# SimonMacLean/NeRF-or-nothing

Hardware: AMD Instinct MI355X
Metric: train rays/sec (128 samples/ray, 8×256 MLP) at 1/2/4/8 MI355X; PSNR vs ref (higher is better)
Workload: dtype f32; 1 GPU; BASELINE configs[1]: 1024-ray global batch x 128+128 samples, 8x256 MLP fwd/bwd + Adam; global_batch=1024, rays_per_gpu=1024, micro_batch=1024, parallelism=dp1, precision=f32

## Files before the change

### include/nof.h

```cpp
#ifndef NOF_H
#define NOF_H

#include <stddef.h>
#include <stdint.h>

#ifdef __cplusplus
extern "C" {
#endif

typedef enum nof_status {
  NOF_OK = 0,
  NOF_ERR_INVALID_ARG = 1,
  NOF_ERR_HIP = 2,
  NOF_ERR_RCCL = 3,
  NOF_ERR_OOM = 4,
  NOF_ERR_UNSUPPORTED = 5
} nof_status;

#define NOF_MAX_LEVELS 4

typedef struct nof_config {
  int32_t device;
  int32_t max_rays;
  int32_t num_levels;
// ... 12 lines not shown
  int32_t precision;
  int32_t grad_buckets;
  int32_t lindisp;
  int32_t ray_shape;
  float density_bias;
  float rgb_padding;
  int32_t stop_level_grad;
  float distortion_loss_mult;
} nof_config;
size_t nof_config_size(void);

enum { NOF_RAY_CONICAL = 0, NOF_RAY_CYLINDRICAL = 1 };

enum {
  NOF_PRECISION_F32 = 0,
  NOF_PRECISION_F32_SPLIT = 1,
  NOF_PRECISION_F16X2 = 2,
  NOF_PRECISION_F32_F16SPLIT = 3,
  NOF_PRECISION_F16 = 4,
  NOF_PRECISION_F16_PRODUCTS = 5
};

void nof_config_default(nof_config* cfg);
const char* nof_last_error(void);
const char* nof_version(void);

typedef struct nof_mipnerf nof_mipnerf;
typedef struct nof_mlp nof_mlp;
typedef struct nof_adam nof_adam;
typedef struct nof_gradcalc nof_gradcalc;

typedef uint64_t (*nof_output_grad_fn)(void* user, uint64_t dev_comp_rgb, int32_t level, float loss_mult_sum,
                                       uint64_t dev_loss_mults);

nof_status nof_mipnerf_create(const nof_config* cfg, nof_mipnerf** out);
nof_status nof_mipnerf_destroy(nof_mipnerf* h);
nof_status nof_mipnerf_get_gradient(nof_mipnerf* h, int32_t n, const float* origins, const float* directions,
                                    const float* radii, const float* nears, const float* fars,
                                    const float* loss_mults, nof_output_grad_fn cb, void* cb_user,
                                    float* const** out_dev_grads);
nof_status nof_mipnerf_get_gradient_device(nof_mipnerf* h, int32_t n, const float* dev_origins,
                                           const float* dev_directions, const float* dev_radii,
                                           const float* dev_nears, const float* dev_fars,
                                           const float* dev_loss_mults, const float* dev_pixels,
                                           float loss_mult_sum, float* const** out_dev_grads);
enum { NOF_GRAD_ACCUMULATE = 1, NOF_GRAD_PUBLISH = 2 };
#define NOF_GRAD_BUCKETS 2
nof_status nof_mipnerf_get_gradient_device_ex(nof_mipnerf* h, int32_t n, const float* dev_origins,
                                              const float* dev_directions, const float* dev_radii,
                                              const float* dev_nears, const float* dev_fars,
                                              const float* dev_loss_mults, const float* dev_pixels,
                                              float loss_mult_sum, uint32_t flags, float* const** out_dev_grads);
typedef void (*nof_grad_bucket_fn)(void* user, int32_t bucket, int32_t nspans, const int64_t* span_offsets,
                                   const int64_t* span_counts);
nof_status nof_mipnerf_set_grad_buckets(nof_mipnerf* h, nof_grad_bucket_fn fn, void* user);
nof_status nof_grad_bucket_spans(int32_t bucket, const int32_t* layer_sizes, int32_t count, int64_t* offsets,
                                 int64_t* counts, int32_t* nspans);
nof_status nof_mipnerf_layer_sizes(nof_mipnerf* h, int32_t* out, int32_t cap, int32_t* count);
nof_status nof_mipnerf_mlp(nof_mipnerf* h, nof_mlp** out);
nof_status nof_mipnerf_set_rng(nof_mipnerf* h, uint64_t seed, uint32_t step, uint32_t ray_base);
nof_status nof_mipnerf_get_rng(nof_mipnerf* h, uint64_t* seed, uint32_t* step, uint32_t* ray_base);

typedef struct nof_level_view {
  int32_t n, samples;
  const float* t;
  const float* weights;
  const float* comp_rgb;
  const float* density;
  const float* rgb;
  const float* density_grad;
  const float* rgb_grad;
} nof_level_view;
nof_status nof_mipnerf_level_view(nof_mipnerf* h, int32_t level, nof_level_view* out);
nof_status nof_mipnerf_cross_view(nof_mipnerf* h, int32_t level, const float** w_grad, const float** t_grad);
nof_status nof_mipnerf_set_ray_grad(nof_mipnerf* h, int32_t enable);
nof_status nof_mipnerf_ray_grad(nof_mipnerf* h, const float** dev_o_grad, const float** dev_d_grad);
nof_status nof_mipnerf_loss(nof_mipnerf* h, float* out);
nof_status nof_mipnerf_distortion_loss(nof_mipnerf* h, float* out);
nof_status nof_mipnerf_set_interlevel_loss(nof_mipnerf* h, float mult);
nof_status nof_mipnerf_interlevel_loss(nof_mipnerf* h, float* out);
enum { NOF_CONTRACT_NONE = 0, NOF_CONTRACT_SPHERE = 1 };
nof_status nof_mipnerf_set_contraction(nof_mipnerf* h, int32_t mode);
nof_status nof_mipnerf_get_contraction(nof_mipnerf* h, int32_t* mode);
typedef struct nof_model_ext {
  uint32_t size;
  int32_t appearance_views, appearance_dim;
} nof_model_ext;
nof_status nof_mipnerf_create_ex(const nof_config* cfg, const nof_model_ext* ext, nof_mipnerf** out);
nof_status nof_mipnerf_appearance(nof_mipnerf* h, float** dev_table, float** dev_grad, int32_t* views, int32_t* dim);
nof_status nof_mipnerf_set_ray_views(nof_mipnerf* h, const int32_t* dev_view_ids);
nof_status nof_mipnerf_set_render_appearance(nof_mipnerf* h, int32_t view);
#define NOF_NUMERIC_FORWARD 1u
#define NOF_NUMERIC_DELTA 2u
nof_status nof_mipnerf_numeric_status(nof_mipnerf* h, uint32_t* flags, int32_t clear);
#define NOF_CHECK_MLP_BLOCK (1u << 0)
#define NOF_CHECK_SAMPLE_IDX (1u << 1)
#define NOF_CHECK_WGRAD_GEOM (1u << 2)
#define NOF_CHECK_GATHER (1u << 3)
#define NOF_CHECK_SELFTEST (1u << 31)
nof_status nof_device_checks(uint32_t* bits, int32_t clear);
nof_status nof_device_checks_selftest(void);

typedef struct nof_render_out {
  int32_t num_levels;
  const float* comp_rgb[NOF_MAX_LEVELS];
  const float* distance[NOF_MAX_LEVELS];
  const float* acc[NOF_MAX_LEVELS];
} nof_render_out;
nof_status nof_mipnerf_render_device(nof_mipnerf* h, int32_t n, const float* dev_origins, const float* dev_dirs,
                                     const float* dev_radii, const float* dev_nears, const float* dev_fars,
                                     int32_t randomized, int32_t white_bkgd, nof_render_out* out);

typedef struct nof_dataset nof_dataset;
typedef struct nof_batch {
  int32_t n;
  float *origins, *directions, *viewdirs;
  float *radii, *nears, *fars, *loss_mults;
  float* pixels;
  int32_t* record_index;
} nof_batch;
nof_status nof_dataset_open(const char* path, int32_t device, nof_dataset** out);
nof_status nof_dataset_open_streaming(const char* path, int32_t device, int64_t max_resident_records,
                                      nof_dataset** out);
nof_status nof_dataset_is_streaming(nof_dataset* ds, int32_t* streaming);
nof_status nof_dataset_from_host(const float* records , int64_t count, int32_t device,
                                 nof_dataset** out);
nof_status nof_dataset_count(nof_dataset* ds, int64_t* count);
nof_status nof_dataset_next(nof_dataset* ds, int32_t n, uint64_t seed, uint32_t step, uint32_t ray_base,
                            void* stream, nof_batch* out, float* loss_mult_sum);
nof_status nof_dataset_destroy(nof_dataset* ds);

nof_status nof_generate_rays(const float* host_poses, int32_t num_views, int32_t width, int32_t height, float focal,
                             float near_, float far_, int32_t ndc, const float* dev_images, float* dev_records,
                             void* stream);
nof_status nof_dataset_generate(const float* host_poses, int32_t num_views, int32_t width, int32_t height, float focal,
                                float near_, float far_, int32_t ndc, const float* dev_images, int32_t device,
                                nof_dataset** out);

nof_status nof_multiscale_layout(int32_t width, int32_t height, float focal, int32_t num_scales,
                                 int32_t disable_multiscale_loss, int32_t num_views, int32_t* w ,
                                 int32_t* h , float* focals , float* lossmults ,
                                 int64_t* firsts , int64_t* count);
nof_status nof_dataset_from_images(const float* host_poses, int32_t num_views, int32_t width, int32_t height,
                                   float focal, float near_, float far_, int32_t ndc, const float* dev_images,
                                   int32_t num_scales, int32_t disable_multiscale_loss, int32_t device,
                                   nof_dataset** out);
nof_status nof_dataset_materialize(nof_dataset* ds, float* dev_records, void* stream);
nof_status nof_recenter_poses(float* host_poses, int32_t num_views);

nof_status nof_checkpoint_save(const char* path, nof_mipnerf* h, nof_adam* adam);
nof_status nof_checkpoint_load(const char* path, nof_mipnerf* h, nof_adam* adam);

typedef struct nof_dp nof_dp;
nof_status nof_dp_unique_id(uint8_t id[128]);
nof_status nof_dp_init_rank(const uint8_t id[128], int32_t world, int32_t rank, int32_t device, nof_dp** out);
nof_status nof_dp_init_rank_timeout(const uint8_t id[128], int32_t world, int32_t rank, int32_t device,
                                    int32_t timeout_ms, nof_dp** out);
nof_status nof_dp_init_all(int32_t ndev, const int32_t* devices, nof_dp** out );
nof_status nof_dp_allreduce(nof_dp* dp, float* dev_buf, int64_t count, void* stream);
nof_status nof_dp_allreduce_grads(nof_dp* dp, nof_mipnerf* h, void* stream);
nof_status nof_dp_allreduce_grads_all(int32_t n, nof_dp* const* dps, nof_mipnerf* const* hs, void* const* streams);
nof_status nof_dp_attach(nof_dp* dp, nof_mipnerf* h, void* comm_stream);
nof_status nof_dp_wait(nof_dp* dp, int32_t timeout_ms);
nof_status nof_dp_step_end(nof_dp* dp, int32_t timeout_ms);
nof_status nof_dp_abort(nof_dp* dp);
nof_status nof_dp_destroy(nof_dp* dp);
// ... 204 lines not shown
```

### nerf-or-nothing_amd/csrc/capi.cpp

```cpp
#include <hip/hip_runtime.h>

#include <cmath>
#include <cstring>
#include <string>
#include <vector>

#include "../../include/nof.h"
#include "host/accelerated.h"
#include "host/trainer.h"
#include "host/dp.h"
#include "kernels/launch.h"

using namespace AcceleratedNeRFUtils;

struct nof_mipnerf { AcceleratedMipNeRF* impl; };
struct nof_mlp { AcceleratedMLP* impl; };
struct nof_adam { AcceleratedAdamOptimizer* impl; };
struct nof_dataset { RayDataset* impl; };
struct nof_gradcalc { AcceleratedGradientCalculator* impl; };

static thread_local std::string g_err;

template <class F>
static nof_status guard(F&& f) {
// ... 187 lines not shown
    *bits = nof::check_unit_sampling(c) | nof::check_unit_mlp_fwd16(c) | nof::check_unit_mlp_bwd16(c) |
            nof::check_unit_wgrad(c) | nof::check_unit_dataset(c) | nof::check_unit_view(c) |
            nof::check_unit_appearance(c);
#else
    (void)clear;
    throw Error(NOF_ERR_UNSUPPORTED, "device checks are compiled only into lib/libnof_check.so (make check)");
#endif
  });
}
nof_status nof_device_checks_selftest(void) {
  return guard([&] {
#ifdef NOF_DEVICE_CHECKS
    NOF_HIP(nof::launch_check_selftest(nullptr));
    NOF_HIP(hipDeviceSynchronize());
#else
    throw Error(NOF_ERR_UNSUPPORTED, "device checks are compiled only into lib/libnof_check.so (make check)");
#endif
  });
}
nof_status nof_mipnerf_set_grad_buckets(nof_mipnerf* h, nof_grad_bucket_fn fn, void* user) {
  return guard([&] {
    ARG(h);
    h->impl->mlp->set_bucket_hook(fn, user);
  });
}
static void copy_sizes(const std::vector<int>& s, int32_t* out, int32_t cap, int32_t* count) {
  if (count) *count = (int32_t)s.size();
  if (out) {
    ARG(cap >= (int32_t)s.size());
    for (size_t i = 0; i < s.size(); ++i) out[i] = s[i];
  }
}
nof_status nof_mipnerf_layer_sizes(nof_mipnerf* h, int32_t* out, int32_t cap, int32_t* count) {
  return guard([&] { ARG(h); copy_sizes(h->impl->GetLayerSizes(), out, cap, count); });
}
nof_status nof_mipnerf_mlp(nof_mipnerf* h, nof_mlp** out) {
  return guard([&] {
    ARG(h && out);
    *out = reinterpret_cast<nof_mlp*>(h->impl->mlp);
  });
}
nof_status nof_mipnerf_set_rng(nof_mipnerf* h, uint64_t seed, uint32_t step, uint32_t ray_base) {
  return guard([&] { ARG(h); h->impl->set_rng(seed, step, ray_base); });
}
nof_status nof_mipnerf_get_rng(nof_mipnerf* h, uint64_t* seed, uint32_t* step, uint32_t* ray_base) {
  return guard([&] { ARG(h && seed && step && ray_base); h->impl->get_rng(seed, step, ray_base); });
}
nof_status nof_mipnerf_level_view(nof_mipnerf* h, int32_t level, nof_level_view* out) {
  return guard([&] { ARG(h && out); *out = h->impl->level_view(level); });
}
nof_status nof_mipnerf_cross_view(nof_mipnerf* h, int32_t level, const float** w_grad, const float** t_grad) {
  return guard([&] { ARG(h && w_grad && t_grad); h->impl->cross_view(level, w_grad, t_grad); });
}
nof_status nof_mipnerf_set_ray_grad(nof_mipnerf* h, int32_t enable) {
  return guard([&] { ARG(h && (enable == 0 || enable == 1)); DEV(h); h->impl->set_ray_grad(enable != 0); });
}
nof_status nof_mipnerf_ray_grad(nof_mipnerf* h, const float** dev_o_grad, const float** dev_d_grad) {
  return guard([&] { ARG(h && dev_o_grad && dev_d_grad); h->impl->ray_grad(dev_o_grad, dev_d_grad); });
}
nof_status nof_mipnerf_loss(nof_mipnerf* h, float* out) {
  return guard([&] { ARG(h && out); DEV(h); *out = h->impl->loss(); });
}
nof_status nof_mipnerf_distortion_loss(nof_mipnerf* h, float* out) {
  return guard([&] { ARG(h && out); DEV(h); *out = h->impl->distortion_loss(); });
}
nof_status nof_mipnerf_set_interlevel_loss(nof_mipnerf* h, float mult) {
  return guard([&] {
    ARG(h);
    if (!(std::isfinite(mult) && mult >= 0.0f))
      throw Error(NOF_ERR_INVALID_ARG, "invalid argument: interlevel_loss_mult must be finite and >= 0");
    DEV(h);
    h->impl->set_interlevel_loss(mult);
  });
}
nof_status nof_mipnerf_interlevel_loss(nof_mipnerf* h, float* out) {
  return guard([&] { ARG(h && out); DEV(h); *out = h->impl->interlevel_loss(); });
}
nof_status nof_mipnerf_set_contraction(nof_mipnerf* h, int32_t mode) {
  return guard([&] {
    ARG(h && (mode == NOF_CONTRACT_NONE || mode == NOF_CONTRACT_SPHERE));
    h->impl->set_contraction(mode);
  });
}
nof_status nof_mipnerf_get_contraction(nof_mipnerf* h, int32_t* mode) {
  return guard([&] { ARG(h && mode); *mode = h->impl->contraction(); });
}
nof_status nof_mipnerf_render_device(nof_mipnerf* h, int32_t n, const float* o, const float* d, const float* radii,
                                     const float* nears, const float* fars, int32_t randomized, int32_t white_bkgd,
                                     nof_render_out* out) {
  return guard([&] {
    ARG(h && out);
    *out = nof_render_out{};
    DEV(h);
    h->impl->Render(n, o, d, radii, nears, fars, randomized, white_bkgd, out);
  });
}
nof_status nof_dataset_open(const char* path, int32_t device, nof_dataset** out) {
  return guard([&] {
    ARG(path && out);
    KEEP_DEVICE;
    auto* d = new nof_dataset{nullptr};
    try { d->impl = new RayDataset(std::string(path), device); } catch (...) { delete d; throw; }
    *out = d;
  });
}
nof_status nof_dataset_open_streaming(const char* path, int32_t device, int64_t max_resident_records,
                                      nof_dataset** out) {
  return guard([&] {
    ARG(path && out && max_resident_records >= 0);
    KEEP_DEVICE;
    auto* d = new nof_dataset{nullptr};
    try { d->impl = new RayDataset(std::string(path), device, max_resident_records); } catch (...) { delete d; throw; }
    *out = d;
  });
}
nof_status nof_dataset_is_streaming(nof_dataset* ds, int32_t* streaming) {
  return guard([&] { ARG(ds && streaming); *streaming = ds->impl->streaming() ? 1 : 0; });
}
nof_status nof_dataset_from_host(const float* records, int64_t count, int32_t device, nof_dataset** out) {
  return guard([&] {
    ARG(records && out);
    KEEP_DEVICE;
    auto* d = new nof_dataset{nullptr};
    try { d->impl = new RayDataset(records, count, device); } catch (...) { delete d; throw; }
    *out = d;
  });
}
nof_status nof_dataset_count(nof_dataset* ds, int64_t* count) {
  return guard([&] { ARG(ds && count); *count = ds->impl->count(); });
}
nof_status nof_dataset_next(nof_dataset* ds, int32_t n, uint64_t seed, uint32_t step, uint32_t ray_base, void* stream,
                            nof_batch* out, float* loss_mult_sum) {
  return guard([&] {
    ARG(ds && out);
    DEV(ds);
    ds->impl->next(n, seed, step, ray_base, (hipStream_t)stream, out, loss_mult_sum);
  });
}
nof_status nof_dataset_destroy(nof_dataset* ds) {
  return guard([&] {
    if (!ds) return;
    DEV(ds);
    delete ds->impl;
    delete ds;
  });
}
nof_status nof_generate_rays(const float* poses, int32_t V, int32_t w, int32_t h, float focal, float near_, float far_,
                             int32_t ndc, const float* dev_images, float* dev_records, void* stream) {
  return guard([&] { generate_rays(poses, V, w, h, focal, near_, far_, ndc, dev_images, dev_records, (hipStream_t)stream); });
}
nof_status nof_dataset_generate(const float* poses, int32_t V, int32_t w, int32_t h, float focal, float near_,
                                float far_, int32_t ndc, const float* dev_images, int32_t device, nof_dataset** out) {
  return guard([&] {
    ARG(poses && out);
    KEEP_DEVICE;
    auto* d = new nof_dataset{nullptr};
    try { d->impl = new RayDataset(poses, V, w, h, focal, near_, far_, ndc, dev_images, device); } catch (...) { delete d; throw; }
    *out = d;
  });
}
nof_status nof_multiscale_layout(int32_t width, int32_t height, float focal, int32_t num_scales,
                                 int32_t disable_multiscale_loss, int32_t num_views, int32_t* w, int32_t* h,
                                 float* focals, float* lossmults, int64_t* firsts, int64_t* count) {
  return guard([&] {
    ARG(w && h && focals && lossmults && firsts && count);
    const nof::MultiscaleLayout L =
// ... 602 lines not shown
```

### nerf-or-nothing_amd/csrc/host/accelerated.cpp

```cpp
#include "accelerated.h"

#include <algorithm>
#include <cmath>
#include <cstring>

#include "../kernels/common.h"
#include "../kernels/mlp_common.h"
#include "../kernels/mlp_h32.h"
#include "trace.h"

namespace AcceleratedNeRFUtils {

using nof::kBlk;

void KernelTimer::enable(uint32_t mask, hipStream_t st) {
  mask_ = mask;
  st_ = st;
  used_ = 0;
  recs_.clear();
  for (int i = 0; i < NOF_NUM_TIMERS; ++i) { tot_ms_[i] = 0.0f; tot_n_[i] = 0; }
}
void KernelTimer::fold() {
  if (!recs_.empty()) NOF_HIP(hipEventSynchronize(recs_.back().b));
  for (const Rec& r : recs_) {
// ... 119 lines not shown
}

AcceleratedMLP::AcceleratedMLP(int deg_point, int deg_view, const nof_config& cfg, int app_views, int app_dim)
    : cfg_(cfg) {
  check_model(cfg, app_views, app_dim);
  if (app_dim > 0) { gV_ = app_views; gG_ = app_dim; }
  NOF_REQUIRE(deg_point == cfg.max_deg_point - cfg.min_deg_point && deg_view == cfg.deg_view,
              "AcceleratedMLP(deg_point, deg_view) must match the config");
  NOF_HIP(hipSetDevice(cfg.device));
  st_ = (hipStream_t)cfg.stream;
  hipDeviceProp_t prop;
  NOF_HIP(hipGetDeviceProperties(&prop, cfg.device));
  num_cu_ = prop.multiProcessorCount;
  aligned_ = cfg.grad_buckets != 0;

  const int D = cfg.net_depth, W = cfg.net_width, Dc = cfg.net_depth_condition, Wc = cfg.net_width_condition;
  const int pos = 6 * (cfg.max_deg_point - cfg.min_deg_point), dir = 3 * (2 * cfg.deg_view + 1);
  const int L = D + Dc + 2;
  out_.resize(L); in_.resize(L); woff_.resize(L); boff_.resize(L);
  for (int l = 0; l < D; ++l) { out_[l] = W; in_[l] = l == 0 ? pos : (l % cfg.skip_layer == 0 ? W + pos : W); }
  out_[D] = 1; in_[D] = W;
  out_[D + 1] = Wc; in_[D + 1] = W + dir + gG_;
  for (int i = 1; i < Dc; ++i) { out_[D + 1 + i] = Wc; in_[D + 1 + i] = Wc; }
  out_[D + 1 + Dc] = 3; in_[D + 1 + Dc] = Wc;
  size_t o = 0;
  for (int l = 0; l < L; ++l) { woff_[l] = (int)o; o += (size_t)out_[l] * in_[l]; }
  for (int l = 0; l < L; ++l) { boff_[l] = (int)o; o += out_[l]; }
  NOF_REQUIRE(o < (size_t)1 << 31, "network too large");
  P_ = o;
  generic_ = any_shape(cfg);
  cross_ = cfg.stop_level_grad == 0 && cfg.num_levels > 1;

  params_.alloc(P_);
  grads_.alloc(P_);
  NOF_HIP(hipMemset(grads_.p, 0, P_ * sizeof(float)));
  std::vector<float> h(P_, 0.0f);
  glorot_host(h.data(), out_.data(), in_.data(), woff_.data(), L, cfg.seed);
  NOF_HIP(hipMemcpy(params_.p, h.data(), P_ * sizeof(float), hipMemcpyHostToDevice));
  for (int l = 0; l < L; ++l) { param_views_.push_back(params_.p + woff_[l]); grad_views_.push_back(grads_.p + woff_[l]); }
  for (int l = 0; l < L; ++l) { param_views_.push_back(params_.p + boff_[l]); grad_views_.push_back(grads_.p + boff_[l]); }

  precision_ = cfg.precision;
  numeric_.alloc(2);
  NOF_HIP(hipMemset(numeric_.p, 0, 2 * sizeof(uint32_t)));
  if (generic_) {
    gD_ = D; gW_ = W; gDc_ = Dc; gWc_ = Wc; gskip_ = cfg.skip_layer; gmin_deg_ = cfg.min_deg_point;
    gP_ = pos; gVd_ = dir;
    gen_alloc();
    return;
  }
  if (precision_ == NOF_PRECISION_F32_SPLIT) {
    wimg_f_.alloc(nof::fwd_image_split_floats<1>() + nof::kFwdTail);
    wimg_b_.alloc(nof::bwd_image_split_floats<1>() + nof::kBwdTail);
  } else if (precision_ == NOF_PRECISION_F16) {
    wimg_f_.alloc(nof::kFwdH32Floats + nof::kFwdTail);
    wimg_b_.alloc(nof::kBwdH32Floats + nof::kBwdTail);
    amax_.alloc(cfg.num_levels);
  } else if (f16_pieces()) {
    wimg_f_.alloc(nof::fwd_image_split_floats<2>() + nof::kFwdTail);
    wimg_b_.alloc(nof::bwd_image_split_floats<2>() + nof::kBwdTail);
    amax_.alloc(cfg.num_levels);
  } else {
    wimg_f_.alloc(nof::kFwdImageFloats);
    wimg_b_.alloc(nof::kBwdImageFloats);
  }

  lv_.resize(cfg.num_levels);
  for (int l = 0; l < cfg.num_levels; ++l) {
    Level& L = lv_[l];
    L.cap = cfg.max_rays * cfg.num_samples[l];
    const size_t nb = (size_t)L.cap / kBlk;
    L.act_in.alloc(nb * nof::kInF * kBlk);
    L.act_h.alloc(8 * nb * 256 * kBlk);
    L.act_h9.alloc(nb * 128 * kBlk);
    L.masks.alloc(nb * nof::kMaskSlots * 256);
    L.zhead.alloc((size_t)L.cap * 4);
    L.sigma.alloc(L.cap);
    L.rgb.alloc((size_t)L.cap * 3);
    L.delta.alloc(8 * nb * 256 * kBlk);
    L.delta9x.alloc(nb * nof::kD9F * kBlk);
    NOF_HIP(hipMemset(L.delta9x.p, 0, L.delta9x.n * sizeof(float)));
    max_M_ = std::max(max_M_, L.cap);
  }
  slab_cap_ = (size_t)(num_cu_ + 64) * 65536;
  slabs_.alloc(slab_cap_);
  bias_slabs_.alloc((size_t)(num_cu_ + 64) * 256);
}

std::vector<int> AcceleratedMLP::get_layer_sizes() const {
  const int L = num_layers();
  std::vector<int> s(2 * L);
  for (int l = 0; l < L; ++l) { s[l] = out_[l] * in_[l]; s[L + l] = out_[l]; }
  return s;
}

bool AcceleratedMLP::pack_weights(const nof::StratArgs* strat) {
  if (generic_) {
    if (f16_products()) {
      NOF_HIP(hipMemsetAsync(amax_.p, 0, lv_.size() * sizeof(uint32_t), st_));
      amax_cleared_ = (1u << lv_.size()) - 1u;
      amax_given_ = 0u;
    }
    return false;
  }
  nof::PackArgs pa;
  if (strat) pa.strat = *strat;
  for (int l = 0; l < kLayers; ++l) { pa.woff[l] = woff_[l]; pa.boff[l] = boff_[l]; }
  if (f16_pieces()) {
    pa.zero = amax_.p;
    pa.nzero = (int)lv_.size();
    amax_cleared_ = (1u << lv_.size()) - 1u;
    amax_given_ = 0u;
  }
  tb(kTPack);
  if (precision_ == NOF_PRECISION_F16)
    NOF_HIP(nof::launch_pack_weights_h32(params_.p, pa, wimg_f_.p, wimg_b_.p, st_));
  else if (precision_ != NOF_PRECISION_F32)
    NOF_HIP(nof::launch_pack_weights_x3(params_.p, pa, wimg_f_.p, wimg_b_.p, f16_pieces() ? 2 : 1, st_));
  else NOF_HIP(nof::launch_pack_weights(params_.p, pa, wimg_f_.p, wimg_b_.p, st_));
  te(kTPack);
  return strat != nullptr;
}

uint32_t* AcceleratedMLP::claim_delta_amax(int level) {
  if (!(f16_pieces() || f16_products()) || level < 0 || level >= (int)lv_.size() || !((amax_cleared_ >> level) & 1u)) return nullptr;
  amax_cleared_ &= ~(1u << level);
  amax_given_ |= 1u << level;
  return amax_.p + level;
}

void AcceleratedMLP::run_forward(int level, const nof::FwdArgs& a0) {
  Level& L = lv_[level];
  nof::FwdArgs a = a0;
  a.split = precision_;
  a.dbias = cfg_.density_bias;
  a.rgb_pad = cfg_.rgb_padding;
  a.rgb_scale = rgb_scale();
  a.wimg = wimg_f_.p;
  a.act_in = L.act_in.p;
  a.act_h = L.act_h.p;
  a.act_h9 = L.act_h9.p;
  a.masks = L.masks.p;
  a.zhead = L.zhead.p;
  a.sigma = L.sigma.p;
  a.rgb = L.rgb.p;
  tb(kTMlpFwd);
  NOF_HIP(nof::launch_mlp_fwd(a, st_));
  te(kTMlpFwd);
}

void AcceleratedMLP::forward_fused(int level, int n, int samples, const float* t, const float* origins,
                                   const float* dirs, const float* radii, bool inference) {
  NOF_REQUIRE(level >= 0 && level < (int)lv_.size(), "level out of range");
  const int M = n * samples;
  NOF_REQUIRE(n > 0 && samples % kBlk == 0 && M <= lv_[level].cap, "batch exceeds the level's capacity");
  lv_[level].M = M; lv_[level].n = n; lv_[level].S = samples;
  if (generic_) {
    NOF_REQUIRE(n <= cfg_.max_rays, "n_rays exceeds max_rays");
    GenLevel& G = gl_[level];
    tb(kTMlpFwd);
    NOF_HIP(nof::launch_cast(n, samples, t, origins, dirs, radii, G.mean.p, G.cov.p, st_, cfg_.ray_shape,
                             contraction_));
    int v;
    NOF_HIP(nof::launch_encode_g(n, samples, G.mean.p, G.cov.p, dirs, gmin_deg_, gP_, gVd_, G.enc_pos.p, G.enc_dir.p,
                                 st_, &v));
    tally(v);
    if (gG_) appearance_gather(level, n);
    te(kTMlpFwd);
    gen_forward(level, G.enc_pos.p, G.enc_dir.p);
    return;
  }
  nof::FwdArgs a{};
  a.M = M; a.S = samples; a.encoded = 0;
  a.no_store = inference ? 1 : 0;
  a.cylinder = cfg_.ray_shape == NOF_RAY_CYLINDRICAL ? 1 : 0;
  a.t = t; a.origins = origins; a.dirs = dirs; a.radii = radii;
  run_forward(level, a);
}

std::pair<float*, float*> AcceleratedMLP::get_output(const float* enc_pos, const float* enc_dir, int level,
                                                     int n_rays, int samples) {
  NOF_REQUIRE(level >= 0 && level < (int)lv_.size(), "level out of range");
  NOF_REQUIRE(enc_pos && enc_dir, "null encoded inputs");
  const int M = n_rays * samples;
  NOF_REQUIRE(n_rays > 0 && samples > 0 && samples % kBlk == 0 && M <= lv_[level].cap,
              "n_rays * samples must be a multiple of 32 within the level's capacity");
  pack_weights();
  lv_[level].M = M; lv_[level].n = n_rays; lv_[level].S = samples;
  if (generic_) {
    NOF_REQUIRE(n_rays <= cfg_.max_rays, "n_rays exceeds max_rays");
    GenLevel& G = gl_[level];
    NOF_HIP(hipMemcpyAsync(G.enc_pos.p, enc_pos, (size_t)M * gP_ * sizeof(float), hipMemcpyDeviceToDevice, st_));
    NOF_HIP(hipMemcpyAsync(G.enc_dir.p, enc_dir, (size_t)n_rays * gVd_ * sizeof(float), hipMemcpyDeviceToDevice,
                           st_));
    if (gG_) appearance_gather(level, n_rays);
    gen_forward(level, G.enc_pos.p, G.enc_dir.p);
    return {lv_[level].sigma.p, lv_[level].rgb.p};
  }
  nof::FwdArgs a{};
  a.M = M; a.S = samples; a.encoded = 1;
  a.enc_pos = enc_pos; a.enc_dir = enc_dir;
  run_forward(level, a);
  return {lv_[level].sigma.p, lv_[level].rgb.p};
}

nof_mlp_debug AcceleratedMLP::debug_view(int level) const {
  NOF_REQUIRE(level >= 0 && level < (int)lv_.size(), "level out of range");
  const Level& L = lv_[level];
  nof_mlp_debug d{};
  d.M = L.M;
  if (generic_) {
    const GenLevel& G = gl_[level];
    d.generic = 1;
    d.gen_h = G.h.p; d.gen_hc = G.hc.p; d.zhead = G.z.p;
    return d;
  }
  d.act_in = L.act_in.p; d.act_h = L.act_h.p; d.act_h9 = L.act_h9.p; d.masks = L.masks.p; d.zhead = L.zhead.p;
  d.delta = L.delta.p; d.delta9x = L.delta9x.p;
  return d;
}

int grad_bucket_spans(const int* sizes, int num_layers, int b, int64_t* off, int64_t* cnt) {
  NOF_REQUIRE(sizes && num_layers >= 1 && b >= 0 && b < AcceleratedMLP::kBuckets, "bad bucket query");
  int64_t w5 = 0, wend = 0, total = 0;
  for (int l = 0; l < num_layers; ++l) {
    if (l < 5) w5 += sizes[l];
    wend += sizes[l];
    total += sizes[l] + sizes[num_layers + l];
  }
  if (b == 0) {
    off[0] = w5; cnt[0] = wend - w5;
    return 1;
  }
  off[0] = 0; cnt[0] = w5;
  off[1] = wend; cnt[1] = total - wend;
  return 2;
}

int AcceleratedMLP::bucket_spans(int b, int64_t* off, int64_t* cnt) const {
  const std::vector<int> s = get_layer_sizes();
  return grad_bucket_spans(s.data(), num_layers(), b, off, cnt);
}

AcceleratedMLP::Schedule& AcceleratedMLP::schedule(int lv0, int lv1, int bucket) {
  NOF_REQUIRE(lv0 >= 0 && lv0 < lv1 && lv1 <= (int)lv_.size(), "bad level range");
  std::vector<int64_t> key{lv0, lv1, bucket, aligned_ ? 1 : 0};
  for (int l = lv0; l < lv1; ++l) key.push_back(lv_[l].M);
  auto it = sched_.find(key);
  if (it != sched_.end()) return it->second;
  const int nlev = lv1 - lv0;
  std::vector<nof::WgProblem> P;
  std::vector<int> pbucket;
  std::vector<int> pnblk;
  struct OutSpec { int prob, row_off, nrows, col_off, ncols; float* dst; int ld, dst_col; float* bias; };
  std::vector<OutSpec> os;
  float* G = grads_.p;
  const bool half = f16_blocks();
  auto at = [&](float* base, size_t off) -> const float* {
    return half ? reinterpret_cast<const float*>(reinterpret_cast<const uint16_t*>(base) + off) : base + off;
// ... 267 lines not shown
      const bool cleared = (amax_cleared_ >> level) & 1u;
      amax_cleared_ &= ~(1u << level);
      NOF_HIP(nof::launch_delta_amax(density_grad, color_grad, L.M, amax_.p + level, st_, numeric_.p, cleared));
    }
    b.amax = amax_.p + level;
  }
  b.dsigma = density_grad; b.drgb = color_grad; b.zhead = L.zhead.p;
  b.masks = L.masks.p;
  b.wimg_b = wimg_b_.p;
  b.delta = L.delta.p; b.delta9x = L.delta9x.p;
  return b;
}

void AcceleratedMLP::run_backward(int level, const float* color_grad, const float* density_grad) {
  const nof::BwdArgs b = bwd_args(level, color_grad, density_grad);
  tb(kTMlpBwd);
  NOF_HIP(nof::launch_mlp_bwd(b, st_));
  te(kTMlpBwd);
}

void AcceleratedMLP::run_backward2(int level, const float* const* color_grads, const float* const* density_grads) {
  nof::BwdArgs b = bwd_args(level, color_grads[0], density_grads[0]);
  const nof::BwdArgs b1 = bwd_args(level + 1, color_grads[1], density_grads[1]);
  b.M1 = b1.M; b.dsigma1 = b1.dsigma; b.drgb1 = b1.drgb; b.zhead1 = b1.zhead; b.amax1 = b1.amax;
  b.masks1 = b1.masks; b.delta1 = b1.delta; b.delta9x1 = b1.delta9x;
  tb(kTMlpBwd);
  NOF_HIP(nof::launch_mlp_bwd(b, st_));
  te(kTMlpBwd);
}

float* const* AcceleratedMLP::wgrad_levels(int lv0, int lv1, int accumulate, bool buckets) {
  if (!buckets) {
    run_wgrad(schedule(lv0, lv1), accumulate);
  } else {
    for (int bk = 0; bk < kBuckets; ++bk) {
      run_wgrad(schedule(lv0, lv1, bk), accumulate);
      int64_t off[2], cnt[2];
      const int ns = bucket_spans(bk, off, cnt);
      TraceRange hr("nof:gradient_bucket_hook");
      hook_(hook_user_, bk, ns, off, cnt);
    }
  }
  return grad_views_.data();
}

float* const* AcceleratedMLP::get_gradient(const float* color_grad, const float* density_grad, int level,
                                           uint32_t flags) {
  NOF_REQUIRE(level >= 0 && level < (int)lv_.size(), "level out of range");
  Level& L = lv_[level];
  NOF_REQUIRE(L.M > 0, "get_gradient before get_output for this level");
  NOF_REQUIRE(color_grad && density_grad, "null output gradients");
  NOF_REQUIRE((flags & ~(uint32_t)(NOF_GRAD_ACCUMULATE | NOF_GRAD_PUBLISH)) == 0, "unknown gradient flags");
  const bool buckets = (flags & NOF_GRAD_PUBLISH) && hook_;
  if (generic_) {
    gen_backward(level, color_grad, density_grad, (level > 0 || (flags & NOF_GRAD_ACCUMULATE)) ? 1 : 0);
    return gen_publish(buckets);
  }
  if (!buckets) (void)schedule(level, level + 1);
  else
    for (int b = 0; b < kBuckets; ++b) (void)schedule(level, level + 1, b);
  run_backward(level, color_grad, density_grad);
  return wgrad_levels(level, level + 1, (level > 0 || (flags & NOF_GRAD_ACCUMULATE)) ? 1 : 0, buckets);
}

float* const* AcceleratedMLP::get_gradient_levels(const float* const* color_grads, const float* const* density_grads,
                                                  uint32_t flags) {
  const int nl = (int)lv_.size();
  NOF_REQUIRE(color_grads && density_grads, "null output gradients");
  for (int l = 0; l < nl; ++l) {
    NOF_REQUIRE(lv_[l].M > 0, "get_gradient before get_output for a level");
    NOF_REQUIRE(color_grads[l] && density_grads[l], "null output gradients");
  }
  NOF_REQUIRE((flags & ~(uint32_t)(NOF_GRAD_ACCUMULATE | NOF_GRAD_PUBLISH)) == 0, "unknown gradient flags");
  const bool buckets = (flags & NOF_GRAD_PUBLISH) && hook_;
  if (generic_) {
    for (int l = 0; l < nl; ++l)
      gen_backward(l, color_grads[l], density_grads[l], (l > 0 || (flags & NOF_GRAD_ACCUMULATE)) ? 1 : 0);
    return gen_publish(buckets);
  }
  if (!buckets) (void)schedule(0, nl);
  else
    for (int b = 0; b < kBuckets; ++b) (void)schedule(0, nl, b);
  int l = 0;
  if (precision_ == NOF_PRECISION_F16)
    for (; l + 1 < nl; l += 2) run_backward2(l, color_grads + l, density_grads + l);
  for (; l < nl; ++l) run_backward(l, color_grads[l], density_grads[l]);
  return wgrad_levels(0, nl, (flags & NOF_GRAD_ACCUMULATE) ? 1 : 0, buckets);
}

static nof::GemmSrc gsrc(const float* p, int64_t si, int64_t sk, int idiv = 1) {
  nof::GemmSrc s;
  s.p = p; s.si = si; s.sk = sk; s.idiv = idiv;
  return s;
}

bool AcceleratedMLP::gen_product(nof::GemmArgs a, int ksplit, bool ws, bool f32) {
  int v;
  if (ksplit == 1) {
    a.kchunk = (a.K1 + a.K2 + 15) / 16 * 16;
    a.slab_stride = 0;
  }
  if (ws && !f16_products() && (!a.G || a.mask_in)) {
    nof::GemmArgs w = a;
    w.G = nullptr;
    if (nof::gemm_ws_fits(w)) {
      NOF_HIP(nof::launch_gemm_ws(w, st_, &v));
      tally(v);
      return true;
    }
  }
  NOF_REQUIRE(a.G || !a.mask_in, "a ReLU-bit mask needs the weight-stationary kernel");
  a.mask_in = nullptr;
  a.mask_out = nullptr;
  if (f16_products() && !f32) {
    NOF_HIP(nof::launch_gemm_h(a, ksplit, st_, &v));
    tally_h(v);
  } else {
    NOF_HIP(nof::launch_gemm(a, ksplit, st_, &v));
    tally(v);
  }
  return false;
}

void AcceleratedMLP::gen_split(int nout, int ncols, int M, int* ksplit, int* kchunk) {
  const int tiles = ((nout + 63) / 64) * ((ncols + 63) / 64);
  int ks = std::max(1, std::min((1024 + tiles - 1) / tiles, M / 64));
  const int kc = ((M + ks - 1) / ks + 15) / 16 * 16;
  *kchunk = kc;
  *ksplit = (M + kc - 1) / kc;
}

void AcceleratedMLP::gen_alloc() {
  const int NL = cfg_.num_levels;
  lv_.resize(NL);
  gl_.resize(NL);
  for (int l = 0; l < NL; ++l) {
    Level& L = lv_[l];
    GenLevel& G = gl_[l];
    L.cap = cfg_.max_rays * cfg_.num_samples[l];
    const size_t M = L.cap;
    G.mean.alloc(3 * M); G.cov.alloc(3 * M);
    G.enc_pos.alloc(M * gP_);
    G.enc_dir.alloc((size_t)cfg_.max_rays * gVd_);
    if (gG_) G.edx.alloc((size_t)cfg_.max_rays * (gVd_ + gG_));
    G.h.alloc((size_t)gD_ * M * gW_);
    G.hc.alloc((size_t)gDc_ * M * gWc_);
    G.z.alloc(4 * M);
    G.mbits.alloc((size_t)(gD_ + gDc_) * M * 4);
    G.mb_ok.assign(gD_ + gDc_, 0);
    L.sigma.alloc(M);
    L.rgb.alloc(3 * M);
    max_M_ = std::max(max_M_, L.cap);
  }
  const size_t Wm = std::max(gW_, gWc_);
  gd0_.alloc((size_t)max_M_ * Wm);
  gd1_.alloc((size_t)max_M_ * Wm);
  gdz_.alloc((size_t)max_M_ * 4);
  gray_.alloc((size_t)cfg_.max_rays * gWc_);
  if (gG_) {
    const size_t T = (size_t)gV_ * gG_;
    app_table_.alloc(T);
    app_grad_.alloc(T);
    app_step_.alloc(T);
    NOF_HIP(hipMemset(app_table_.p, 0, T * sizeof(float)));
    NOF_HIP(hipMemset(app_grad_.p, 0, T * sizeof(float)));
    gdapp_.alloc((size_t)cfg_.max_rays * gG_);
  }
// ... 376 lines not shown
  t_.resize(L); w_.resize(L); C_.resize(L); dsig_.resize(L); drgb_.resize(L); loss_rays_.resize(L);
  acc_.resize(L); dist_.resize(L);
  for (int l = 0; l < L; ++l) {
    const size_t S = cfg.num_samples[l];
    t_[l].alloc(N * (S + 1)); w_[l].alloc(N * S); C_[l].alloc(3 * N); acc_[l].alloc(N); dist_[l].alloc(N);
    dsig_[l].alloc(N * S); drgb_[l].alloc(3 * N * S); loss_rays_[l].alloc(N);
  }
  dist_rays_.alloc(N);
  cross_ = mlp->cross();
  if (cross_) {
    q_.resize(L); dtr_.resize(L); dtb_.resize(L); dt_.resize(L);
    for (int l = 0; l < L; ++l) {
      const size_t S = cfg.num_samples[l];
      if (l + 1 < L) q_[l].alloc(N * S);
      if (l >= 1) { dtr_[l].alloc(N * (S + 1)); dt_[l].alloc(N * (S + 1)); }
      if (l >= 1 && l + 1 < L) dtb_[l].alloc(N * (S + 1));
    }
  }
}

AcceleratedMipNeRF::~AcceleratedMipNeRF() {
  if (attached_dp) {
    mlp->set_bucket_hook(nullptr, nullptr);
    dp_model_destroyed(attached_dp, this);
  }
  delete mlp;
}

void AcceleratedMipNeRF::set_ray_views(const int32_t* ids) {
  NOF_REQUIRE(has_appearance(), "the model has no appearance embeddings (nof_mipnerf_create_ex)");
  mlp->set_ray_views(ids);
}

void AcceleratedMipNeRF::require_ray_views() const {
  NOF_REQUIRE(!has_appearance() || mlp->ray_views(),
              "a gradient step of an appearance model needs its ray views (nof_mipnerf_set_ray_views before every "
              "step)");
}

float* const* AcceleratedMipNeRF::GetGradient(int n, const float* origins, const float* directions,
                                              const float* radii, const float* nears, const float* fars,
                                              const float* loss_mults, nof_output_grad_fn cb, void* user) {
  NOF_REQUIRE(n > 0 && n <= cfg_.max_rays, "ray count out of range");
  NOF_REQUIRE(origins && directions && radii && nears && fars && loss_mults && cb, "null argument");
  require_ray_views();
  float msum = 0.0f;
  for (int i = 0; i < n; ++i) msum += loss_mults[i];
  NOF_HIP(hipMemcpyAsync(o_.p, origins, 3 * n * sizeof(float), hipMemcpyHostToDevice, st_));
  NOF_HIP(hipMemcpyAsync(d_.p, directions, 3 * n * sizeof(float), hipMemcpyHostToDevice, st_));
  NOF_HIP(hipMemcpyAsync(radii_.p, radii, n * sizeof(float), hipMemcpyHostToDevice, st_));
  NOF_HIP(hipMemcpyAsync(nears_.p, nears, n * sizeof(float), hipMemcpyHostToDevice, st_));
  NOF_HIP(hipMemcpyAsync(fars_.p, fars, n * sizeof(float), hipMemcpyHostToDevice, st_));
  NOF_HIP(hipMemcpyAsync(lm_.p, loss_mults, n * sizeof(float), hipMemcpyHostToDevice, st_));
  return run(n, o_.p, d_.p, radii_.p, nears_.p, fars_.p, lm_.p, nullptr, msum, cb, user, NOF_GRAD_PUBLISH);
}

float* const* AcceleratedMipNeRF::GetGradientDevice(int n, const float* o, const float* d, const float* radii,
                                                    const float* nears, const float* fars, const float* loss_mults,
                                                    const float* pixels, float msum, uint32_t flags) {
  NOF_REQUIRE(n > 0 && n <= cfg_.max_rays, "ray count out of range");
  NOF_REQUIRE(o && d && radii && nears && fars && loss_mults && pixels, "null argument");
  NOF_REQUIRE(msum > 0.0f, "loss_mult_sum must be > 0");
  NOF_REQUIRE((flags & ~(uint32_t)(NOF_GRAD_ACCUMULATE | NOF_GRAD_PUBLISH)) == 0, "unknown gradient flags");
  require_ray_views();
  return run(n, o, d, radii, nears, fars, loss_mults, pixels, msum, nullptr, nullptr, flags);
}

float* const* AcceleratedMipNeRF::run(int n, const float* o, const float* d, const float* radii, const float* nears,
                                      const float* fars, const float* lm, const float* pix, float msum,
                                      nof_output_grad_fn cb_in, void* user, uint32_t flags) {
  static const char* const kFwd[] = {"nof:level0_forward", "nof:level1_forward", "nof:level2_forward",
                                     "nof:level3_forward"};
  static const char* const kBwd[] = {"nof:backward"};
  const int L = cfg_.num_levels;
  TraceRange step_range("nof:get_gradient");
  struct ViewScope {
    AcceleratedMLP* m;
    ~ViewScope() { m->set_ray_views(nullptr); m->set_appearance_job(nullptr, 0, 0); }
  } view_scope{mlp};
  if (has_appearance()) mlp->set_appearance_job(mlp->ray_views(), (flags & NOF_GRAD_ACCUMULATE) ? 1 : 0, L);
  nof::StratArgs sa;
  sa.n = n; sa.S = cfg_.num_samples[0]; sa.nears = nears; sa.fars = fars; sa.randomized = cfg_.randomized;
  sa.lindisp = cfg_.lindisp; sa.seed = seed_; sa.step = step_; sa.ray_base = ray_base_; sa.t = t_[0].p;
  const bool sampled = mlp->pack_weights(&sa);
  for (int lv = 0; lv < L; ++lv) {
    TraceRange lr(kFwd[lv & 3]);
    const int S = cfg_.num_samples[lv];
    if (lv == 0 && !sampled) {
      timer.begin(kTSample);
      NOF_HIP(nof::launch_sample_stratified(n, S, nears, fars, cfg_.randomized, seed_, step_, 0, ray_base_,
                                            t_[0].p, st_, cfg_.lindisp));
      timer.end(kTSample);
    }
    mlp->forward_fused(lv, n, S, t_[lv].p, o, d, radii);
    const bool cb = cb_in || cross_;
    if (lv + 1 < L || cb) timer.begin(kTRenderFwd);
    if (lv + 1 < L) {
      nof::RenderPdfArgs ra{};
      ra.n = n; ra.S = S; ra.sigma = mlp->density(lv); ra.rgb = mlp->rgb(lv); ra.t = t_[lv].p; ra.d = d;
      ra.white = cfg_.white_bkgd; ra.C = C_[lv].p; ra.w = w_[lv].p; ra.nonfinite = mlp->numeric_flags();
      ra.S_out = cfg_.num_samples[lv + 1]; ra.padding = cfg_.resample_padding; ra.randomized = cfg_.randomized;
      ra.seed = seed_; ra.step = step_; ra.level = (uint32_t)(lv + 1); ra.ray_base = ray_base_; ra.t_out = t_[lv + 1].p;
      NOF_HIP(nof::launch_render_fwd_pdf(ra, st_));
    } else if (cb) {
      NOF_HIP(nof::launch_render_fwd(n, S, mlp->density(lv), mlp->rgb(lv), t_[lv].p, d, cfg_.white_bkgd, C_[lv].p,
                                     w_[lv].p, st_, nullptr, nullptr, mlp->numeric_flags()));
    }
    if (lv + 1 < L || cb) timer.end(kTRenderFwd);
  }
  struct JobScope {
    AcceleratedMLP* m;
    ~JobScope() { m->set_ray_grad_job(nullptr); }
  } job_scope{mlp};
  if (mlp->ray_grad()) {
    AcceleratedMLP::RayGradJob job;
    job.n = n; job.o = o; job.d = d; job.radius = radii;
    for (int lv = 0; lv < L; ++lv) job.t[lv] = t_[lv].p;
    mlp->set_ray_grad_job(&job);
    ray_grad_valid_ = true;
  }
  if (cross_) {
    float* const* g = run_cross(n, o, d, radii, nears, fars, lm, pix, msum, cb_in, user, flags);
    dist_valid_ = true;
    prop_valid_ = true;
    last_n_ = n;
    last_fused_ = cb_in == nullptr;
    ++step_;
    return g;
  }
  nof_output_grad_fn cb = cb_in;
  if (prop_mult_ > 0.0f && L >= 2) {
    run_interlevel(n, d, nears, fars, lm, pix, msum, cb, user);
  } else {
    nof::RenderBwdArgs ra{};
    ra.n = n; ra.d = d; ra.white = cfg_.white_bkgd; ra.pix = pix; ra.lossmult = lm; ra.msum = msum;
    ra.nonfinite = mlp->numeric_flags();
    const float dmult = cfg_.distortion_loss_mult;
    if (dmult > 0.0f) { ra.nears = nears; ra.fars = fars; ra.lindisp = cfg_.lindisp; }
    int nb = 0;
    auto flush = [&]() {
      if (!nb) return;
      timer.begin(kTRenderBwd);
      NOF_HIP(nof::launch_render_bwd(ra, nb, st_));
      timer.end(kTRenderBwd);
      nb = 0;
    };
    for (int lv = 0; lv < L; ++lv) {
      const int S = cfg_.num_samples[lv];
      const float* g = nullptr;
      if (cb) {
        g = reinterpret_cast<const float*>(cb(user, (uint64_t)(uintptr_t)C_[lv].p, lv, msum, (uint64_t)(uintptr_t)lm));
        NOF_REQUIRE(g != nullptr, "output-gradient callback returned null");
      }
      if (nb && (cb || S != ra.S || nb == nof::kRenderMaxLevels)) flush();
      ra.S = S;
      nof::RenderBwdLevel& R = ra.lv[nb++];
      R.sigma = mlp->density(lv); R.rgb = mlp->rgb(lv); R.t = t_[lv].p; R.C = C_[lv].p; R.g_ext = g;
      R.lam = lv < L - 1 ? cfg_.coarse_loss_mult : 1.0f;
      R.dsigma = dsig_[lv].p; R.drgb = drgb_[lv].p; R.loss_rays = cb ? nullptr : loss_rays_[lv].p;
      R.amax = mlp->claim_delta_amax(lv);
      R.dist_mult = lv == L - 1 ? dmult : 0.0f;
      R.dist_rays = lv == L - 1 && dmult > 0.0f ? dist_rays_.p : nullptr;
      if (lv == L - 1 && !cb) {
        ra.fwd_last = 1; ra.fwd_C = C_[lv].p; ra.fwd_w = w_[lv].p;
      }
      if (cb) flush();
    }
// ... 368 lines not shown
```

### nerf-or-nothing_amd/csrc/host/accelerated.h

```cpp
#pragma once
#include <hip/hip_runtime.h>

#include <array>
#include <map>
#include <stdexcept>
#include <string>
#include <vector>

#include "../../../include/nof.h"
#include "../kernels/launch.h"

namespace AcceleratedNeRFUtils {

struct Error : std::runtime_error {
  nof_status code;
  Error(nof_status c, const std::string& m) : std::runtime_error(m), code(c) {}
};

#define NOF_HIP(expr)                                                                                    \
  do {                                                                                                   \
    hipError_t _e = (expr);                                                                              \
    if (_e != hipSuccess)                                                                                \
      throw ::AcceleratedNeRFUtils::Error(_e == hipErrorOutOfMemory ? NOF_ERR_OOM : NOF_ERR_HIP,         \
                                          std::string(#expr) + ": " + hipGetErrorString(_e));            \
// ... 11 lines not shown
  DevBuf() = default;
  explicit DevBuf(size_t count) { alloc(count); }
  void alloc(size_t count) {
    release();
    n = count;
    if (count) NOF_HIP(hipMalloc(&p, count * sizeof(T)));
  }
  void release() {
    if (p) (void)hipFree(p);
    p = nullptr;
    n = 0;
  }
  ~DevBuf() { release(); }
  DevBuf(const DevBuf&) = delete;
  DevBuf& operator=(const DevBuf&) = delete;
  DevBuf(DevBuf&& o) noexcept : p(o.p), n(o.n) { o.p = nullptr; o.n = 0; }
  DevBuf& operator=(DevBuf&& o) noexcept {
    if (this != &o) { release(); p = o.p; n = o.n; o.p = nullptr; o.n = 0; }
    return *this;
  }
};

class KernelTimer {
 public:
  void enable(uint32_t mask, hipStream_t st);
  bool on() const { return mask_ != 0; }
  void begin(int id);
  void end(int id);
  void read(float* ms, int* launches, int cap);
  ~KernelTimer();

 private:
  hipEvent_t get();
  void fold();
  static constexpr size_t kMaxRecs = 4096;
  float tot_ms_[NOF_NUM_TIMERS] = {};
  int tot_n_[NOF_NUM_TIMERS] = {};
  uint32_t mask_ = 0;
  hipStream_t st_ = nullptr;
  std::vector<hipEvent_t> pool_;
  size_t used_ = 0;
  struct Rec { int id; hipEvent_t a, b; };
  std::vector<Rec> recs_;
  hipEvent_t open_[NOF_NUM_TIMERS] = {};
};

enum TimerId { kTPack = 0, kTSample, kTMlpFwd, kTRenderFwd, kTRenderBwd, kTMlpBwd, kTWgrad, kTWgradReduce };

class AcceleratedMLP {
 public:
  static constexpr int kLayers = 11;
  static constexpr int kTensors = 22;
  static constexpr int kMaxLayers = 16;
  int num_layers() const { return (int)out_.size(); }
  bool generic() const { return generic_; }

  AcceleratedMLP(int deg_point, int deg_view, const nof_config& cfg, int app_views = 0,
                 int app_dim = 0);
  ~AcceleratedMLP() = default;

  std::vector<int> get_layer_sizes() const;
  std::pair<float*, float*> get_output(const float* enc_pos, const float* enc_dir, int level, int n_rays,
                                       int samples);
  float* const* get_gradient(const float* color_grad, const float* density_grad, int level, uint32_t flags = 0);
  float* const* get_gradient_levels(const float* const* color_grads, const float* const* density_grads,
                                    uint32_t flags);
  static constexpr int kBuckets = 2;
  void set_bucket_hook(nof_grad_bucket_fn fn, void* user) {
    hook_ = fn;
    hook_user_ = user;
    aligned_ = fn != nullptr || cfg_.grad_buckets != 0;
  }
  bool has_bucket_hook() const { return hook_ != nullptr; }
  int bucket_spans(int b, int64_t* off, int64_t* cnt) const;

  float* const* allParams() const { return param_views_.data(); }
  float* const* allGradients() const { return grad_views_.data(); }
  float* flat_params() const { return params_.p; }
  float* flat_grads() const { return grads_.p; }
  int64_t num_params() const { return (int64_t)P_; }

  void forward_fused(int level, int n, int samples, const float* t, const float* origins, const float* dirs,
                     const float* radii, bool inference = false);
  bool pack_weights(const nof::StratArgs* strat = nullptr);
  const float* density(int level) const { return lv_[level].sigma.p; }
  const float* rgb(int level) const { return lv_[level].rgb.p; }
  KernelTimer* timer = nullptr;
  hipStream_t stream() const { return st_; }
  int device() const { return cfg_.device; }
  nof_mlp_debug debug_view(int level) const;
  const uint32_t* gen_dispatch() const { return disp_; }
  void clear_gen_dispatch() { for (uint32_t& c : disp_) c = 0; }
  const uint32_t* gen_dispatch_h() const { return disp_h_; }
  void clear_gen_dispatch_h() { for (uint32_t& c : disp_h_) c = 0; }
  uint32_t* numeric_flags() const { return numeric_.p; }
  uint32_t* claim_delta_amax(int level);
  bool cross() const { return cross_; }
  void gradient_level_cross(int level, const float* color_grad, const float* density_grad, int accumulate,
                            const float** denc);
  float* const* publish_cross(uint32_t flags) { return gen_publish((flags & NOF_GRAD_PUBLISH) && hook_); }
  const float* enc_pos(int level) const { return gl_[level].ep; }
  struct RayGradJob {
    int n = 0;
    const float *o = nullptr, *d = nullptr, *radius = nullptr;
    const float* t[NOF_MAX_LEVELS] = {};
    bool first = true;
  };
  void set_ray_grad(bool on);
  bool ray_grad() const { return ray_grad_; }
  void set_ray_grad_job(const RayGradJob* job) { rg_job_ = job ? *job : RayGradJob(); }
  const float* ray_o_grad() const { return rg_o_.p; }
  const float* ray_d_grad() const { return rg_d_.p; }
  void set_contraction(int mode);
  int contraction() const { return contraction_; }
  int appearance_views() const { return gV_; }
  int appearance_dim() const { return gG_; }
  float* appearance_table() const { return app_table_.p; }
  float* appearance_grad() const { return app_grad_.p; }
  void set_ray_views(const int32_t* ids) { app_ids_ = ids; }
  const int32_t* ray_views() const { return app_ids_; }
  void set_render_appearance(int view);
  void set_appearance_job(const int32_t* ids, int accumulate, int levels) {
    app_job_ = AppJob{ids, accumulate, levels, true};
  }

 private:
  struct AppJob {
    const int32_t* ids = nullptr;
    int accumulate = 0;
    int left = 0;
    bool first = true;
  };
  struct Schedule {
    DevBuf<nof::WgProblem> probs;
    DevBuf<nof::WgItem> items;
    DevBuf<int> item_ptr;
    DevBuf<int64_t> slab_off;
    DevBuf<nof::WgOut> outs;
    int nouts = 0, max_elems = 0, num_wg = 0;
    int lv0 = 0;
  };
  struct Level {
    int cap = 0, M = 0, n = 0, S = 0;
    DevBuf<float> act_in, act_h, act_h9, zhead, sigma, rgb;
    DevBuf<float> delta, delta9x;
    DevBuf<uint32_t> masks;
  };
  void run_forward(int level, const nof::FwdArgs& a);
  nof::BwdArgs bwd_args(int level, const float* color_grad, const float* density_grad);
  void run_backward(int level, const float* color_grad, const float* density_grad);
  void run_backward2(int level, const float* const* color_grads, const float* const* density_grads);
  Schedule& schedule(int lv0, int lv1, int bucket = -1);
  std::map<std::vector<int64_t>, Schedule> sched_;
  void run_wgrad(Schedule& sc, int accumulate);
  float* const* wgrad_levels(int lv0, int lv1, int accumulate, bool buckets);
  nof_grad_bucket_fn hook_ = nullptr;
  bool aligned_ = false;
  void* hook_user_ = nullptr;
  void tb(int id) { if (timer) timer->begin(id); }
  void te(int id) { if (timer) timer->end(id); }

  nof_config cfg_;
  hipStream_t st_;
  int num_cu_ = 256;
  int precision_ = 0;
  bool f16_pieces() const {
    return precision_ == NOF_PRECISION_F16X2 || precision_ == NOF_PRECISION_F32_F16SPLIT || precision_ == NOF_PRECISION_F16;
  }
  bool f16_products() const { return precision_ == NOF_PRECISION_F16_PRODUCTS; }
  bool f16_blocks() const { return precision_ == NOF_PRECISION_F16X2 || precision_ == NOF_PRECISION_F16; }
  float rgb_scale() const { return 1.0f + 2.0f * cfg_.rgb_padding; }
  size_t P_ = 0;
  std::vector<int> out_, in_, woff_, boff_;

  bool generic_ = false;
  int gD_ = 0, gW_ = 0, gDc_ = 0, gWc_ = 0, gskip_ = 0, gmin_deg_ = 0, gP_ = 0, gVd_ = 0;
  struct GenLevel {
    DevBuf<float> mean, cov, enc_pos, enc_dir;
    DevBuf<float> edx;
    DevBuf<float> h, hc, z;
    const float *ep = nullptr, *ed = nullptr;
    DevBuf<uint32_t> mbits;
    std::vector<char> mb_ok;
  };
  bool gen_product(nof::GemmArgs a, int ksplit = 1, bool ws = false, bool f32 = false);
  uint32_t disp_[nof::kGvCount] = {};
  uint32_t disp_h_[nof::kGhCount] = {};
  void tally(int variant, int launches = 1) { if (variant >= 0) disp_[variant] += (uint32_t)launches; }
  void tally_h(int variant) { if (variant >= 0) ++disp_h_[variant]; }
  std::vector<GenLevel> gl_;
  DevBuf<float> gd0_, gd1_, gdz_, gslab_;
  DevBuf<float> gray_;
  void gen_alloc();
  void gen_forward(int level, const float* enc_pos, const float* enc_dir);
  void gen_backward(int level, const float* color_grad, const float* density_grad, int accumulate,
                    bool want_denc = false);
  bool cross_ = false;
  DevBuf<float> gd2_, gdenc_, gdenc_part_;
  void denc_alloc(int first_level);
  bool ray_grad_ = false;
  int contraction_ = NOF_CONTRACT_NONE;
  RayGradJob rg_job_;
  DevBuf<float> gddir_, rg_o_, rg_d_;
  int gV_ = 0, gG_ = 0;
  DevBuf<float> app_table_, app_grad_;
  DevBuf<float> app_step_;
  DevBuf<float> gdapp_;
  const int32_t* app_ids_ = nullptr;
  int app_const_ = -1;
  AppJob app_job_;
  void appearance_gather(int level, int n);
  size_t* wg_need_ = nullptr;
  std::vector<nof::SlabJob> wg_jobs_;
  size_t wg_off_ = 0;
  void gen_wgrad(float* dst, int64_t ld, const float* dz, int64_t ldz, int nout, nof::GemmSrc x, int ncols, int M,
                 int accumulate, float* bias_dst = nullptr, const uint32_t* scale = nullptr);
  static void gen_split(int nout, int ncols, int M, int* ksplit, int* kchunk);
  float* const* gen_publish(bool buckets);
  DevBuf<float> params_, grads_, wimg_f_, wimg_b_;
  std::vector<float*> param_views_, grad_views_;
  std::vector<Level> lv_;
  int max_M_ = 0;
  DevBuf<float> slabs_, bias_slabs_;
  DevBuf<uint32_t> amax_;
  uint32_t amax_cleared_ = 0;
  uint32_t amax_given_ = 0;
  DevBuf<uint32_t> numeric_;
  size_t slab_cap_ = 0;
};

void dp_model_destroyed(nof_dp* dp, class AcceleratedMipNeRF* model);

int grad_bucket_spans(const int* sizes, int num_layers, int b, int64_t* off, int64_t* cnt);

void check_model(const nof_config& cfg, int app_views, int app_dim);

class AcceleratedMipNeRF {
 public:
  explicit AcceleratedMipNeRF(const nof_config& cfg, int app_views = 0, int app_dim = 0);
  ~AcceleratedMipNeRF();
  AcceleratedMLP* mlp;

  float* const* GetGradient(int n, const float* origins, const float* directions, const float* radii,
                            const float* nears, const float* fars, const float* loss_mults, nof_output_grad_fn cb,
                            void* user);
  float* const* GetGradientDevice(int n, const float* o, const float* d, const float* radii, const float* nears,
                                  const float* fars, const float* loss_mults, const float* pixels, float msum,
                                  uint32_t flags = NOF_GRAD_PUBLISH);
  std::vector<int> GetLayerSizes() const { return mlp->get_layer_sizes(); }

  void set_rng(uint64_t seed, uint32_t step, uint32_t ray_base) { seed_ = seed; step_ = step; ray_base_ = ray_base; }
  void get_rng(uint64_t* seed, uint32_t* step, uint32_t* ray_base) const { *seed = seed_; *step = step_; *ray_base = ray_base_; }
  nof_level_view level_view(int level) const;
  void cross_view(int level, const float** w_grad, const float** t_grad) const;
  void set_ray_grad(bool on);
  void ray_grad(const float** o_grad, const float** d_grad) const;
  float loss();
  float distortion_loss();
  void set_interlevel_loss(float mult);
  float interlevel_loss();
  void set_contraction(int mode) { mlp->set_contraction(mode); }
  int contraction() const { return mlp->contraction(); }
  bool has_appearance() const { return mlp->appearance_dim() > 0; }
  void set_ray_views(const int32_t* ids);
  void set_render_appearance(int view) { mlp->set_render_appearance(view); }
  void require_ray_views() const;
  uint32_t numeric_status(bool clear);
  void Render(int n, const float* o, const float* d, const float* radii, const float* nears, const float* fars,
              int randomized, int white_bkgd, nof_render_out* out);
  KernelTimer timer;
  nof_dp* attached_dp = nullptr;

 private:
  float* const* run(int n, const float* o, const float* d, const float* radii, const float* nears,
                    const float* fars, const float* lm, const float* pix, float msum, nof_output_grad_fn cb,
                    void* user, uint32_t flags);
  nof_config cfg_;
  hipStream_t st_;
  uint64_t seed_;

 public:
  const nof_config& config() const { return cfg_; }
  int device() const { return cfg_.device; }

 private:
  uint32_t step_ = 0, ray_base_ = 0;
  int last_n_ = 0;
  bool last_fused_ = false;
  bool ray_grad_valid_ = false;
  bool dist_valid_ = false;
  DevBuf<float> dist_rays_;
  float prop_mult_ = 0.0f;
  bool prop_valid_ = false;
  std::vector<DevBuf<float>> prop_rays_;
  DevBuf<float> o_, d_, radii_, nears_, fars_, lm_, pix_;
  std::vector<DevBuf<float>> t_, w_, C_, dsig_, drgb_, loss_rays_, acc_, dist_;
  void launch_interlevel_level(int n, int l, const float* lm, float msum, int accumulate);
  void run_interlevel(int n, const float* d, const float* nears, const float* fars, const float* lm, const float* pix,
                      float msum, nof_output_grad_fn cb, void* user);
  bool cross_ = false;
  std::vector<DevBuf<float>> q_, dtr_, dtb_, dt_;
  float* const* run_cross(int n, const float* o, const float* d, const float* radii, const float* nears,
// ... 51 lines not shown
```

### nerf-or-nothing_amd/csrc/kernels/adam.hip

```cpp
#include "common.h"
#include "launch.h"
#include "resample.h"
#include "mlp_common.h"
#include "mlp_h32.h"

#pragma clang fp contract(off)

namespace nof {

static int strat_blocks(const StratArgs& z) { return z.n > 0 ? (z.n * (z.S + 1) + 255) / 256 : 0; }

__global__ void k_adam(int64_t n, float* __restrict__ p, const float* __restrict__ g, float* __restrict__ m,
                       float* __restrict__ v, float lr, float inv1, float inv2) {
  const float b1 = 0.9f, b2 = 0.999f;
  for (int64_t i = (int64_t)blockIdx.x * blockDim.x + threadIdx.x; i < n; i += (int64_t)gridDim.x * blockDim.x) {
    const float gi = g[i];
    const float mi = b1 * m[i] + (1.0f - b1) * gi;
    const float vi = b2 * v[i] + (1.0f - b2) * gi * gi;
    m[i] = mi;
    v[i] = vi;
    const float mh = mi * inv1, vh = vi * inv2;
    p[i] = p[i] - lr * mh * (1.0f / sqrtf(vh + 1e-8f));
  }
}

hipError_t launch_adam(int64_t n, float* p, const float* g, float* m, float* v, float lr, float inv1, float inv2,
                       hipStream_t st) {
  if (n <= 0) return hipSuccess;
  int64_t blocks = (n + 255) / 256;
  if (blocks > 2048) blocks = 2048;
  hipLaunchKernelGGL(k_adam, dim3((unsigned)blocks), dim3(256), 0, st, n, p, g, m, v, lr, inv1, inv2);
  return hipGetLastError();
}

__device__ inline void adam_at(const AdamSegs& s, int64_t i, float*& p, const float*& g) {
  int lo = 0, hi = s.n - 1;
  while (lo < hi) {
    const int mid = (lo + hi + 1) >> 1;
    if (s.off[mid] <= i) lo = mid;
    else hi = mid - 1;
  }
  p = s.p[lo] + (i - s.off[lo]);
  g = s.g[lo] + (i - s.off[lo]);
}
__device__ inline float adam_g1(float g, float p, float wdc) { return wdc != 0.0f ? g + wdc * p : g; }
__device__ inline float adam_g2(float g1, float mv) { return mv > 0.0f ? fminf(fmaxf(g1, -mv), mv) : g1; }

template <bool MAX>
__device__ inline double adam_block_reduce(double x, double* sh) {
#pragma unroll
  for (int o = 32; o > 0; o >>= 1) {
    const double y = __shfl_xor(x, o, 64);
    x = MAX ? fmax(x, y) : x + y;
  }
  if ((threadIdx.x & 63) == 0) sh[threadIdx.x >> 6] = x;
  __syncthreads();
  return MAX ? fmax(fmax(fmax(sh[0], sh[1]), sh[2]), sh[3]) : ((sh[0] + sh[1]) + sh[2]) + sh[3];
}

__global__ __launch_bounds__(256) void k_adam_stats(int64_t n, const AdamSegs s, AdamOpts o,
                                                    double* __restrict__ part) {
  __shared__ double sh[4][4];
  double s1 = 0.0, s2 = 0.0, sp = 0.0, mx = 0.0;
  for (int64_t i = (int64_t)blockIdx.x * blockDim.x + threadIdx.x; i < n; i += (int64_t)gridDim.x * blockDim.x) {
    float* pp;
    const float* gp;
    adam_at(s, i, pp, gp);
    const float pi = *pp;
    const float g1 = adam_g1(*gp, pi, o.wdc), g2 = adam_g2(g1, o.grad_max_val);
    s1 += (double)g1 * (double)g1;
    s2 += (double)g2 * (double)g2;
    sp += (double)pi * (double)pi;
    mx = fmax(mx, (double)fabsf(g1));
  }
  s1 = adam_block_reduce<false>(s1, sh[0]);
  s2 = adam_block_reduce<false>(s2, sh[1]);
  sp = adam_block_reduce<false>(sp, sh[2]);
  mx = adam_block_reduce<true>(mx, sh[3]);
  if (threadIdx.x == 0) {
    part[0 * kAdamStatBlocks + blockIdx.x] = s1;
    part[1 * kAdamStatBlocks + blockIdx.x] = s2;
    part[2 * kAdamStatBlocks + blockIdx.x] = sp;
    part[3 * kAdamStatBlocks + blockIdx.x] = mx;
  }
}

template <bool MOD>
__global__ __launch_bounds__(256) void k_adam_opt(int64_t n, const AdamSegs s, float* __restrict__ m,
                                                  float* __restrict__ v, float lr, float inv1, float inv2, AdamOpts o,
                                                  const double* __restrict__ part, int nb, AdamStepStats* rec,
                                                  int32_t iteration) {
  __shared__ double sh[4][4];
  const float b1 = 0.9f, b2 = 0.999f;
// ... 16 lines not shown
        rec->iteration = iteration;
      }
    }
  }
  for (int64_t i = (int64_t)blockIdx.x * blockDim.x + threadIdx.x; i < n; i += (int64_t)gridDim.x * blockDim.x) {
    float* pp;
    const float* gp;
    adam_at(s, i, pp, gp);
    const float pi = *pp;
    float gi = *gp;
    if (MOD) gi = adam_g2(adam_g1(gi, pi, o.wdc), o.grad_max_val) * scale;
    const float mi = b1 * m[i] + (1.0f - b1) * gi;
    const float vi = b2 * v[i] + (1.0f - b2) * gi * gi;
    m[i] = mi;
    v[i] = vi;
    const float mh = mi * inv1, vh = vi * inv2;
    *pp = pi - lr * mh * (1.0f / sqrtf(vh + 1e-8f));
  }
}

static int adam_stat_blocks(int64_t total) {
  const int64_t b = (total + 255) / 256;
  return (int)(b < kAdamStatBlocks ? b : kAdamStatBlocks);
}
hipError_t launch_adam_stats(int64_t total, const AdamSegs& s, const AdamOpts& o, double* partials, hipStream_t st) {
  if (total <= 0) return hipSuccess;
  if (s.n < 1 || s.n > kAdamMaxSegs || s.off[0] != 0 || s.off[s.n] != total) return hipErrorInvalidValue;
  hipLaunchKernelGGL(k_adam_stats, dim3((unsigned)adam_stat_blocks(total)), dim3(256), 0, st, total, s, o, partials);
  return hipGetLastError();
}
hipError_t launch_adam_opt(int64_t total, const AdamSegs& s, float* m, float* v, float lr, float inv1, float inv2,
                           const AdamOpts& o, bool modify, const double* partials, AdamStepStats* record,
                           int32_t iteration, hipStream_t st) {
  if (total <= 0) return hipSuccess;
  if (s.n < 1 || s.n > kAdamMaxSegs || s.off[0] != 0 || s.off[s.n] != total) return hipErrorInvalidValue;
  int64_t blocks = (total + 255) / 256;
  if (blocks > 2048) blocks = 2048;
  const int nb = adam_stat_blocks(total);
  if (modify)
    hipLaunchKernelGGL(k_adam_opt<true>, dim3((unsigned)blocks), dim3(256), 0, st, total, s, m, v, lr, inv1, inv2, o,
                       partials, nb, record, iteration);
  else
    hipLaunchKernelGGL(k_adam_opt<false>, dim3((unsigned)blocks), dim3(256), 0, st, total, s, m, v, lr, inv1, inv2, o,
                       partials, nb, record, iteration);
  return hipGetLastError();
}

struct LoopPtrs { float* p[kLoopMax]; };
__global__ void k_loopback_sum(int k, LoopPtrs b, int64_t n) {
  for (int64_t i = (int64_t)blockIdx.x * blockDim.x + threadIdx.x; i < n; i += (int64_t)gridDim.x * blockDim.x) {
    float s = b.p[0][i];
    for (int j = 1; j < k; ++j) s += b.p[j][i];
    for (int j = 0; j < k; ++j) b.p[j][i] = s;
  }
}
hipError_t launch_loopback_sum(int k, float* const* bufs, int64_t n, hipStream_t st) {
  if (k < 1 || k > kLoopMax) return hipErrorInvalidValue;
  if (n <= 0) return hipSuccess;
  LoopPtrs b{};
  for (int j = 0; j < k; ++j) b.p[j] = bufs[j];
  int64_t blocks = (n + 255) / 256;
  if (blocks > 2048) blocks = 2048;
  hipLaunchKernelGGL(k_loopback_sum, dim3((unsigned)blocks), dim3(256), 0, st, k, b, n);
  return hipGetLastError();
}

__device__ inline int layer_out(int l) { return l < 8 ? 256 : (l == 8 ? 1 : (l == 9 ? 128 : 3)); }
__device__ inline int layer_in(int l) {
  return l == 0 ? 96 : (l == 4 ? 352 : (l < 8 ? 256 : (l == 8 ? 256 : (l == 9 ? 283 : 128))));
}

__device__ inline void fwd_slice(int s, int& l, int& col) {
  if (s < 3) { l = 0; col = 32 * s; }
  else if (s < 27) { l = 1 + (s - 3) / 8; col = 32 * ((s - 3) % 8); }
  else if (s < 38) { l = 4; col = 32 * (s - 27); }
  else if (s < 62) { l = 5 + (s - 38) / 8; col = 32 * ((s - 38) % 8); }
  else { l = 9; col = 32 * (s - 62); }
}
__device__ inline void bwd_slice(int s, int& l, int& o) {
  if (s < 4) { l = 9; o = 32 * s; }
  else { l = 7 - (s - 4) / 8; o = 32 * ((s - 4) % 8); }
}

__global__ void k_pack_weights(const float* __restrict__ P, PackArgs pa, float* __restrict__ wf,
                               float* __restrict__ wb) {
  if ((int)blockIdx.x >= pa.pack_blocks) {
    const StratArgs& z = pa.strat;
    stratified_t(((int)blockIdx.x - pa.pack_blocks) * (int)blockDim.x + (int)threadIdx.x, z.n, z.S, z.nears, z.fars,
                 z.randomized, z.lindisp, z.seed, z.step, 0, z.ray_base, z.t);
    return;
  }
  const int64_t gid = (int64_t)blockIdx.x * blockDim.x + threadIdx.x;
  const int64_t nf = (int64_t)kFwdImageFloats, nb = (int64_t)kBwdImageFloats;
  if (gid < nf) {
    const int64_t slices = (int64_t)kFwdSlices * kSliceFloats;
    float v = 0.0f;
    if (gid < slices) {
      const int s = (int)(gid / kSliceFloats);
      const int e = (int)(gid - (int64_t)s * kSliceFloats);
      const int r = e >> 5, pc = e & 31;
      const int c = ((((pc >> 2) ^ ((r >> 1) & 7)) << 2) | (pc & 3));
      int l, col;
      fwd_slice(s, l, col);
      const int in = layer_in(l);
      if (r < layer_out(l) && col + c < in) v = P[pa.woff[l] + (int64_t)r * in + col + c];
    } else {
      const int t = (int)(gid - slices);
      if (t < kFwdTailW8) {
        const int l = t / 256, x = t % 256;
        v = x < layer_out(l) ? P[pa.boff[l] + x] : 0.0f;
      } else if (t < kFwdTailW10) {
        v = P[pa.woff[8] + (t - kFwdTailW8)];
      } else if (t < kFwdTailW9d) {
        v = P[pa.woff[10] + (t - kFwdTailW10)];
      } else {
        const int o = (t - kFwdTailW9d) / 32, k = (t - kFwdTailW9d) % 32;
        v = k < kDirIn ? P[pa.woff[9] + (int64_t)o * 283 + 256 + k] : 0.0f;
      }
    }
    wf[gid] = v;
  } else if (gid < nf + nb) {
    const int64_t b = gid - nf;
    const int64_t slices = (int64_t)kBwdSlices * kSliceFloats;
    float v = 0.0f;
    if (b < slices) {
      const int s = (int)(b / kSliceFloats);
      const int e = (int)(b - (int64_t)s * kSliceFloats);
      const int i = e >> 5, pc = e & 31;
      const int c = ((((pc >> 2) ^ ((i >> 1) & 7)) << 2) | (pc & 3));
      int l, o;
      bwd_slice(s, l, o);
      v = P[pa.woff[l] + (int64_t)(o + c) * layer_in(l) + i];
    } else {
      const int t = (int)(b - slices);
      v = t < kBwdTailW10 ? P[pa.woff[8] + t] : P[pa.woff[10] + (t - kBwdTailW10)];
    }
    wb[b] = v;
  }
}

__device__ inline float fwd_tail_value(const float* __restrict__ P, const PackArgs& pa, int t) {
  if (t < kFwdTailW8) {
    const int l = t / 256, x = t % 256;
    return x < layer_out(l) ? P[pa.boff[l] + x] : 0.0f;
  }
  if (t < kFwdTailW10) return P[pa.woff[8] + (t - kFwdTailW8)];
  if (t < kFwdTailW9d) return P[pa.woff[10] + (t - kFwdTailW10)];
  const int o = (t - kFwdTailW9d) / 32, k = (t - kFwdTailW9d) % 32;
  return k < kDirIn ? P[pa.woff[9] + (int64_t)o * 283 + 256 + k] : 0.0f;
}
__device__ inline float bwd_tail_value(const float* __restrict__ P, const PackArgs& pa, int t) {
  return t < kBwdTailW10 ? P[pa.woff[8] + t] : P[pa.woff[10] + (t - kBwdTailW10)];
}
template <int P>
__device__ inline typename SplitMode<P>::V2 split_piece2(float w, int piece) {
  typename SplitMode<P>::V2 o[SplitMode<P>::NP];
  split2<P>(w, w, o);
  typename SplitMode<P>::V2 r = o[0];
#pragma unroll
  for (int p = 1; p < SplitMode<P>::NP; ++p) r = piece == p ? o[p] : r;
  return r;
}

template <int P>
__global__ void k_pack_weights_x3(const float* __restrict__ P_, PackArgs pa, float* __restrict__ wf,
                                  float* __restrict__ wb) {
  if ((int)blockIdx.x >= pa.pack_blocks) {
    const StratArgs& z = pa.strat;
    stratified_t(((int)blockIdx.x - pa.pack_blocks) * (int)blockDim.x + (int)threadIdx.x, z.n, z.S, z.nears, z.fars,
                 z.randomized, z.lindisp, z.seed, z.step, 0, z.ray_base, z.t);
    return;
  }
  constexpr int NP = SplitMode<P>::NP;
  constexpr int kChunks = split_slice_floats<P>() / 4;
  const float* __restrict__ Pp = P_;
  const int64_t gid = (int64_t)blockIdx.x * blockDim.x + threadIdx.x;
  if (gid < pa.nzero) pa.zero[gid] = 0u;
  const int64_t nfc = (int64_t)kFwdSlices * kChunks, nbc = (int64_t)kBwdSlices * kChunks;
  if (gid < nfc + nbc) {
    const bool fwd = gid < nfc;
    const int64_t c = fwd ? gid : gid - nfc;
    const int slice = (int)(c / kChunks), q = (int)(c % kChunks);
    const int lane = q & 63, rest = q >> 6;
    const int piece = P == 2 ? rest / 16 : rest % NP, so = P == 2 ? rest % 16 : rest / NP;
    const int row = P == 2 ? 16 * so + (lane & 15) : (so & 7) * 32 + (lane & 31);
    int l, base;
    if (fwd) fwd_slice(slice, l, base);
    else bwd_slice(slice, l, base);
    const int in = layer_in(l);
    typename SplitMode<P>::V8 out;
#pragma unroll
    for (int j = 0; j < 8; ++j) {
      const int kf = P == 2 ? 16 * (j >> 2) + 4 * (lane >> 4) + (j & 3)
                            : 16 * (so >> 3) + 8 * (j >> 2) + 4 * (lane >> 5) + (j & 3);
      float w;
      if (fwd) w = (row < layer_out(l) && base + kf < in) ? Pp[pa.woff[l] + (int64_t)row * in + base + kf] : 0.0f;
      else w = Pp[pa.woff[l] + (int64_t)(base + kf) * in + row];
      out[j] = split_piece2<P>(w, piece)[0];
    }
    float* dst = (fwd ? wf : wb) + (size_t)slice * split_slice_floats<P>() + (size_t)q * 4;
    *reinterpret_cast<typename SplitMode<P>::V8*>(dst) = out;
  } else {
    const int t = (int)(gid - nfc - nbc);
    if (t < kFwdTail) wf[fwd_image_split_floats<P>() + t] = fwd_tail_value(Pp, pa, t);
    else if (t < kFwdTail + kBwdTail)
      wb[bwd_image_split_floats<P>() + (t - kFwdTail)] = bwd_tail_value(Pp, pa, t - kFwdTail);
  }
}
hipError_t launch_pack_weights_x3(const float* params, const PackArgs& pa, float* wimg_f, float* wimg_b,
                                  int precision, hipStream_t st) {
  const int chunks = precision == 2 ? split_slice_floats<2>() / 4 : split_slice_floats<1>() / 4;
  const int64_t total = (int64_t)(kFwdSlices + kBwdSlices) * chunks + kFwdTail + kBwdTail;
  PackArgs a = pa;
  a.pack_blocks = (int)((total + 255) / 256);
  const dim3 grid((unsigned)(a.pack_blocks + strat_blocks(pa.strat)));
  if (precision == 2) hipLaunchKernelGGL(k_pack_weights_x3<2>, grid, dim3(256), 0, st, params, a, wimg_f, wimg_b);
  else hipLaunchKernelGGL(k_pack_weights_x3<1>, grid, dim3(256), 0, st, params, a, wimg_f, wimg_b);
  return hipGetLastError();
}

__global__ void k_pack_weights_h32(const float* __restrict__ P, PackArgs pa, float* __restrict__ wf,
                                   float* __restrict__ wb) {
  if ((int)blockIdx.x >= pa.pack_blocks) {
    const StratArgs& z = pa.strat;
    stratified_t(((int)blockIdx.x - pa.pack_blocks) * (int)blockDim.x + (int)threadIdx.x, z.n, z.S, z.nears, z.fars,
                 z.randomized, z.lindisp, z.seed, z.step, 0, z.ray_base, z.t);
    return;
  }
  const int64_t gid = (int64_t)blockIdx.x * blockDim.x + threadIdx.x;
  if (gid < pa.nzero) pa.zero[gid] = 0u;
  const int64_t nfc = (int64_t)(kFwdFrags + kStreamPad) * 64, nbc = (int64_t)(kBwdFrags + kStreamPad) * 64;
  if (gid < nfc + nbc) {
    const bool fwd = gid < nfc;
    const int64_t q = fwd ? gid : gid - nfc;
    const int g = (int)(q >> 6), lane = (int)(q & 63), x = lane & 31, h = lane >> 5;
    f16x8 out;
#pragma unroll
    for (int j = 0; j < 8; ++j) out[j] = (_Float16)0.0f;
    if (g < (fwd ? kFwdFrags : kBwdFrags)) {
      int start = 0, si = 0;
      H32Seg sg = fwd ? fwd_seg(0) : bwd_seg(0);
      while (g >= start + sg.nk * sg.nc) {
        start += sg.nk * sg.nc;
        ++si;
        sg = fwd ? fwd_seg(si) : bwd_seg(si);
      }
      const int c = (g - start) / sg.nk, kk = (g - start) % sg.nk, l = sg.layer, in = layer_in(l);
#pragma unroll
      for (int j = 0; j < 8; ++j) {
        float w;
        if (fwd) {
          const int col = kk < 16 ? kfeat(kk, h, j) : 256 + kfeat(kk - 16, h, j);
          const bool dens = l == 9 && c == 4;
          const int ll = dens ? 8 : l, row = dens ? x : 32 * c + x;
          w = row < layer_out(ll) ? P[pa.woff[ll] + (int64_t)row * layer_in(ll) + col] : 0.0f;
        } else if (kk < 16 && (l != 9 || kk < 8)) {
          w = P[pa.woff[l] + (int64_t)kfeat(kk, h, j) * in + 32 * c + x];
        } else {
          w = (kk == 8 && kfeat(0, h, j) == 0) ? P[pa.woff[8] + 32 * c + x] : 0.0f;
        }
        out[j] = (_Float16)w;
      }
    }
    *reinterpret_cast<f16x8*>((fwd ? wf : wb) + (size_t)q * 4) = out;
  } else {
    const int t = (int)(gid - nfc - nbc);
    if (t < kFwdTail) wf[kFwdH32Floats + t] = fwd_tail_value(P, pa, t);
    else if (t < kFwdTail + kBwdTail) wb[kBwdH32Floats + (t - kFwdTail)] = bwd_tail_value(P, pa, t - kFwdTail);
  }
}
hipError_t launch_pack_weights_h32(const float* params, const PackArgs& pa, float* wimg_f, float* wimg_b,
                                   hipStream_t st) {
  const int64_t total = (int64_t)(kFwdFrags + kBwdFrags + 2 * kStreamPad) * 64 + kFwdTail + kBwdTail;
  PackArgs a = pa;
  a.pack_blocks = (int)((total + 255) / 256);
  hipLaunchKernelGGL(k_pack_weights_h32, dim3((unsigned)(a.pack_blocks + strat_blocks(pa.strat))), dim3(256), 0, st,
                     params, a, wimg_f, wimg_b);
  return hipGetLastError();
}

hipError_t launch_pack_weights(const float* params, const PackArgs& pa, float* wimg_f, float* wimg_b, hipStream_t st) {
  const int64_t total = (int64_t)kFwdImageFloats + (int64_t)kBwdImageFloats;
  PackArgs a = pa;
  a.pack_blocks = (int)((total + 255) / 256);
  hipLaunchKernelGGL(k_pack_weights, dim3((unsigned)(a.pack_blocks + strat_blocks(pa.strat))), dim3(256), 0, st,
                     params, a, wimg_f, wimg_b);
  return hipGetLastError();
}

}
```

### nerf-or-nothing_amd/csrc/kernels/launch.h

```cpp
#pragma once
#include <hip/hip_runtime.h>
#include <stdint.h>

namespace nof {

uint32_t check_unit_sampling(bool clear);
uint32_t check_unit_mlp_fwd16(bool clear);
uint32_t check_unit_mlp_bwd16(bool clear);
uint32_t check_unit_wgrad(bool clear);
uint32_t check_unit_dataset(bool clear);
uint32_t check_unit_view(bool clear);
uint32_t check_unit_appearance(bool clear);
hipError_t launch_check_selftest(hipStream_t st);

hipError_t launch_sample_stratified(int n, int S, const float* nears, const float* fars, int randomized,
                                    uint64_t seed, uint32_t step, uint32_t level, uint32_t ray_base, float* t,
                                    hipStream_t st, int lindisp = 0);
hipError_t launch_sample_pdf(int n, int S_in, const float* t_in, const float* w, int S_out, float padding,
                             int randomized, uint64_t seed, uint32_t step, uint32_t level, uint32_t ray_base,
                             float* t_out, int32_t* idx_out, hipStream_t st);
hipError_t launch_cast(int n, int S, const float* t, const float* o, const float* d, const float* radius,
                       float* mean, float* cov, hipStream_t st, int ray_shape = 0, int contraction = 0);
hipError_t launch_encode(int n, int S, const float* mean, const float* cov, const float* d, float* enc_pos,
                         float* enc_dir, hipStream_t st);
// ... 27 lines not shown
  uint32_t* amax;
  float dist_mult = 0.0f;
  float* dist_rays = nullptr;
};
struct RenderBwdArgs {
  int n, S, white;
  const float *d, *pix, *lossmult;
  float msum;
  uint32_t* nonfinite;
  RenderBwdLevel lv[kRenderMaxLevels];
  int fwd_last = 0;
  float *fwd_C = nullptr, *fwd_w = nullptr;
  const float *nears = nullptr, *fars = nullptr;
  int lindisp = 0;
};
hipError_t launch_render_bwd(const RenderBwdArgs& a, int nlev, hipStream_t st);
hipError_t launch_output_gradient(int n, const float* C, const float* pix, const float* lossmult,
                                  float loss_mult_sum, float lam, float* g, hipStream_t st);

struct RenderBwdXArgs {
  int n, S, white;
  const float *d, *pix, *lossmult;
  float msum;
  uint32_t* nonfinite;
  const float *sigma, *rgb, *t, *C, *g_ext;
  float lam;
  float *dsigma, *drgb, *loss_rays;
  const float* q;
  float* t_grad;
  int fwd;
  float *fwd_C, *fwd_w;
  float dist_mult;
  float* dist_rays;
  const float *nears, *fars;
  int lindisp;
};
hipError_t launch_render_bwd_x(const RenderBwdXArgs& a, hipStream_t st);

struct EncodeGradArgs {
  int n, S, P, min_deg, cylinder;
  const float *t, *o, *d, *radius, *enc, *denc;
  const float *add0, *add1;
  float* t_grad;
  int contract;
};
hipError_t launch_encode_grad(const EncodeGradArgs& a, hipStream_t st);
struct SamplePdfGradArgs {
  int n, S_in, S_out;
  const float *t_in, *w;
  float padding;
  int randomized;
  uint64_t seed;
  uint32_t step, level, ray_base;
  const float* t_out_grad;
  float *w_grad, *t_in_grad;
};
hipError_t launch_sample_pdf_grad(const SamplePdfGradArgs& a, hipStream_t st);

struct InterlevelArgs {
  int n, S_prop, S_tgt, accumulate;
  const float *t_prop, *w_prop, *t_tgt, *w_tgt, *lossmult;
  float msum, mult;
  float *w_grad, *rays;
};
hipError_t launch_interlevel(const InterlevelArgs& a, hipStream_t st);

struct RayGradArgs {
  int n, S, P, min_deg, cylinder, Vd, accumulate;
  const float *t, *o, *d, *radius, *enc, *denc, *sigma, *dsigma;
  const float *enc_dir, *ddir;
  float *o_grad, *d_grad;
  int contract;
};
hipError_t launch_ray_grad(const RayGradArgs& a, hipStream_t st);

struct FwdArgs {
  int M, S, encoded;
  int no_store;
  int split;
  int cylinder;
  float dbias = -1.0f, rgb_scale = 1.002f, rgb_pad = 0.001f;
  const float *t, *origins, *dirs, *radii;
  const float *enc_pos, *enc_dir;
  const float* wimg;
  float* act_in;
  float* act_h;
  float* act_h9;
  uint32_t* masks;
  float* zhead;
  float* sigma;
  float* rgb;
};
hipError_t launch_mlp_fwd(const FwdArgs& a, hipStream_t st);

struct BwdArgs {
  int M;
  int split;
  const float *dsigma, *drgb, *zhead;
  const uint32_t* amax;
  float dbias = -1.0f, rgb_scale = 1.002f;
  const uint32_t* masks;
  const float* wimg_b;
  float* delta;
  float* delta9x;
  int M1;
  const float *dsigma1, *drgb1, *zhead1;
  const uint32_t *amax1, *masks1;
  float *delta1, *delta9x1;
};
hipError_t launch_mlp_bwd(const BwdArgs& a, hipStream_t st);
hipError_t launch_delta_amax(const float* dsigma, const float* drgb, int M, uint32_t* amax, hipStream_t st,
                             uint32_t* nonfinite = nullptr, bool cleared = false);
hipError_t launch_mlp_fwd16(const FwdArgs& a, hipStream_t st);
hipError_t launch_mlp_bwd16(const BwdArgs& a, hipStream_t st);
hipError_t launch_mlp_fwd_h32(const FwdArgs& a, hipStream_t st);
int device_cus();
hipError_t launch_mlp_bwd_h32(const BwdArgs& a, hipStream_t st);

struct WgProblem {
  const float* A; const float* B;
  int FA, a_row0, ntr;
  int FB, b_col0, ntc;
  int shape;
  int ntc1;
  const float* B2; int FB2, b2_col0, ntc2;
  const float* B3; int FB3, b3_col0, ntc3;
  int level;
};
struct WgItem { int prob, kb0, kb1; int slab; };
int wgrad_reduce_threads(int nrows, int ncols, int col_off);
constexpr int kWgMaxLevels = 4;
struct WgOut {
  int item0, nitems;
  int lev_items[kWgMaxLevels];
  int nlev;
  int row_off, nrows, col_off, ncols;
  float* dst; int ld, dst_col;
  float* bias_dst;
  int prob;
};
hipError_t launch_wgrad(const WgProblem* probs, const WgItem* items, const int* item_ptr, int num_wg,
                        const int64_t* slab_off, float* slabs, float* bias_slabs, hipStream_t st);
int wgrad_shape(int ntr, int ntc, int* cost2);
int wgrad_block_cost(int ntr, int ntc, int* shape);
int wgrad_x3_grid_cols();
hipError_t launch_wgrad_x3(const WgProblem* probs, const WgItem* items, const int* item_ptr, int num_wg,
                           const int64_t* slab_off, float* slabs, float* bias_slabs, int precision, hipStream_t st);
hipError_t launch_wgrad_reduce(const WgOut* outs, int nouts, int max_elems, const WgItem* items,
                               const WgProblem* probs, const int64_t* slab_off, const float* slabs,
                               const float* bias_slabs, int accumulate, const uint32_t* amax, hipStream_t st);

struct GemmSrc {
  const float* p = nullptr;
  int64_t si = 0, sk = 0;
  int idiv = 1;
};
struct GemmArgs {
  int M = 0, N = 0, K1 = 0, K2 = 0;
  GemmSrc A1, A2, B1, B2;
  const float* bias = nullptr;
  int relu = 0;
  const float* G = nullptr; int64_t gi = 0, gj = 0;
  float* C = nullptr; int64_t ci = 0, cj = 0;
  int kchunk = 0; int64_t slab_stride = 0;
  float* rowsum = nullptr;
  const uint32_t* mask_in = nullptr;
// ... 71 lines not shown
  int64_t first[kMaxScales];
  int64_t count;
};
hipError_t launch_pyramid_level(float* pyr, const MultiscaleLayout& L, int s, hipStream_t st);
hipError_t launch_materialize(const float* poses, const float* pyr, const MultiscaleLayout& L, float near, float far,
                              int ndc, float* records, hipStream_t st);
hipError_t launch_gather_rays(const float* poses, const float* pyr, const MultiscaleLayout& L, float near, float far,
                              int ndc, int n, uint64_t seed, uint32_t step, uint32_t ray_base, float* o, float* d,
                              float* vd, float* radius, float* nears, float* fars, float* lm, float* pix, int* idx_out,
                              float* lm_sum, hipStream_t st);
hipError_t launch_pose_grad(const MultiscaleLayout& L, int n, const int* idx, const float* o_grad, const float* d_grad,
                            float* pose_grad, int accumulate, hipStream_t st);
hipError_t launch_batch_views(const MultiscaleLayout& L, int n, const int* idx, int* views, hipStream_t st);

hipError_t launch_appearance_gather(int n, int vd, int dim, int views, const float* enc_dir, const float* table,
                                    const int* ids, int const_view, float* out, hipStream_t st);
hipError_t launch_appearance_grad(int n, int dim, int views, const int* ids, const float* d_app, const float* partial,
                                  float* d_table, int accumulate, hipStream_t st);

struct ViewRayArgs {
  const float* poses;
  float pose[12];
  int use_pose, view, num_views;
  int w, h;
  float focal, near, far;
  int ndc, p0, n;
  float *o, *d, *radius, *nears, *fars;
};
hipError_t launch_view_rays(const ViewRayArgs& a, hipStream_t st);
constexpr int kViewMaxLevels = 4;
constexpr int kViewStoreBlock = 256;
inline int view_store_blocks(int n) { return (n + kViewStoreBlock - 1) / kViewStoreBlock; }
struct ViewStoreArgs {
  int num_levels;
  const float* comp_rgb[kViewMaxLevels];
  const float *dist_in, *acc_in;
  float* rgb[kViewMaxLevels];
  float *distance, *acc;
  const float* gt;
  double* partials;
  int block0, blocks;
  int p0, n, npix;
  int view, num_views;
};
hipError_t launch_view_store(const ViewStoreArgs& a, hipStream_t st);
hipError_t launch_view_final(const double* partials, int blocks, int num_levels, double* sums, hipStream_t st);

hipError_t image_metrics(const float* a, const float* b, int W, int H, float max_val, float* psnr, float* ssim,
                         hipStream_t st);

constexpr int kLoopMax = 8;
hipError_t launch_loopback_sum(int k, float* const* bufs, int64_t n, hipStream_t st);
hipError_t launch_adam(int64_t n, float* p, const float* g, float* m, float* v, float lr, float inv1, float inv2,
                       hipStream_t st);
constexpr int kAdamStatBlocks = 256;
constexpr int kAdamMaxSegs = 64;
struct AdamSegs {
  int n = 0;
  int64_t off[kAdamMaxSegs + 1] = {};
  float* p[kAdamMaxSegs] = {};
  const float* g[kAdamMaxSegs] = {};
};
struct AdamOpts {
  float grad_max_norm = 0.0f, grad_max_val = 0.0f;
  float wdc = 0.0f;
};
struct AdamStepStats {
  float weight_l2, grad_norm, grad_abs_max, grad_norm_clipped, clip_scale;
  int32_t iteration;
};
hipError_t launch_adam_stats(int64_t total, const AdamSegs& s, const AdamOpts& o, double* partials, hipStream_t st);
hipError_t launch_adam_opt(int64_t total, const AdamSegs& s, float* m, float* v, float lr, float inv1, float inv2,
                           const AdamOpts& o, bool modify, const double* partials, AdamStepStats* record,
                           int32_t iteration, hipStream_t st);
struct StratArgs {
  int n = 0, S = 0;
  const float* nears = nullptr;
  const float* fars = nullptr;
  int randomized = 0, lindisp = 0;
  uint64_t seed = 0;
  uint32_t step = 0, ray_base = 0;
  float* t = nullptr;
};
struct PackArgs {
  int woff[11]; int boff[11];
  uint32_t* zero = nullptr; int nzero = 0;
  StratArgs strat;
  int pack_blocks = 0;
};
hipError_t launch_pack_weights(const float* params, const PackArgs& pa, float* wimg_f, float* wimg_b, hipStream_t st);
hipError_t launch_pack_weights_h32(const float* params, const PackArgs& pa, float* wimg_f, float* wimg_b,
                                   hipStream_t st);
hipError_t launch_pack_weights_x3(const float* params, const PackArgs& pa, float* wimg_f, float* wimg_b,
                                  int precision, hipStream_t st);

}
```

### nerf-or-nothing_amd/csrc/kernels/mlp_bwd16.hip

```cpp
#include "common.h"
#include "launch.h"
#include "mlp16.h"

namespace nof {


template <bool kDensity, class ST, bool kSplit = false>
struct BwdEpi16 {
  static constexpr int kVmPerPart = 4;
  const f32x4 (&acc)[16];
  float (&bin)[16][4];
  const ST& bst;
  const int g;
  const float* w8;
  float dzs;
  __amdgpu_buffer_rsrc_t dst_blk;
  uint2 mk;
  f32x4 wnext;

  __device__ __forceinline__ BwdEpi16(const f32x4 (&acc_)[16], float (&bin_)[16][4], const ST& bst_, int lane)
      : acc(acc_), bin(bin_), bst(bst_), g(lane >> 4) {}
  template <class E>
  __device__ __forceinline__ void begin(const uint2* mask, E* dst_blk_, const float* w8_ = nullptr, float dzs_ = 0.0f) {
    mk = *mask;
    dst_blk = blk_rsrc_t(dst_blk_);
    if constexpr (kDensity) {
      w8 = w8_ + 4 * g;
      dzs = dzs_;
      wnext = *reinterpret_cast<const f32x4*>(w8);
    }
  }
  __device__ __forceinline__ void operator()(int t) {
    f32x4 w4;
    if constexpr (kDensity) {
      w4 = wnext;
      if (t + 1 < 16) wnext = *reinterpret_cast<const f32x4*>(w8 + 16 * (t + 1));
    }
    float v[4];
#pragma unroll
    for (int r = 0; r < 4; ++r) {
      v[r] = acc[t][r];
      if constexpr (kDensity) v[r] = __builtin_fmaf(w4[r], dzs, v[r]);
      v[r] = mask16_apply(mk, t, r, v[r]);
    }
    put_tile<kSplit, true>(bin, t, v, bst, dst_blk);
  }
  __device__ __forceinline__ void tile01() {
    (*this)(0);
    (*this)(1);
  }
};

template <int P>
__global__ __launch_bounds__(kMlp16Threads, 1) void k_mlp_bwd16(BwdArgs a) {
  typedef typename Store16<P, true>::T ST;
  typedef typename Store16<P, true>::E AE;
  __shared__ __attribute__((aligned(16))) float lds[ring16_floats<P>() + 256];
  float* w8_lds = lds + ring16_floats<P>();
  const int tid = threadIdx.x, lane = tid & 63, g = lane >> 4, j = lane & 15;
  const int wave = __builtin_amdgcn_readfirstlane(tid >> 6);
  const int half = wave & 1;
  const ST bst(lane, half);
  const int nblk = a.M / kBlk;
  const int blk_raw = blockIdx.x * 4 + (wave >> 1);
  const int blk = blk_raw < nblk ? blk_raw : nblk - 1;
  const int m = blk * kBlk + 16 * half + j;
  NOF_DCHECK(a.M % kBlk == 0 && blk >= 0 && blk < nblk, kChkMlpBlock);
  const float* tail = a.wimg_b + (size_t)kBwdSlices * kSliceFloats;
  const size_t layer_stride = (size_t)nblk * kWidth * kBlk;
  uint32_t* masks = const_cast<uint32_t*>(a.masks);

  ring16_prologue(a.wimg_b, lds, tid);

  const f32x4 zh = reinterpret_cast<const f32x4*>(a.zhead)[m];
  float dzs = a.dsigma[m] * sigmoid_f(zh[0] + a.dbias);
  float dzc[3];
#pragma unroll
  for (int c = 0; c < 3; ++c) {
    const float s = sigmoid_f(zh[1 + c]);
    dzc[c] = a.drgb[(size_t)m * 3 + c] * (s * (1.0f - s)) * a.rgb_scale;
  }
  if constexpr (P >= 2) {
    const float sc = delta_scale(a.amax, false);
    dzs *= sc;
#pragma unroll
    for (int c = 0; c < 3; ++c) dzc[c] *= sc;
  }
  const __amdgpu_buffer_rsrc_t d9 = blk_rsrc_t(reinterpret_cast<AE*>(a.delta9x) + (size_t)blk * kD9F * kBlk);
#pragma unroll
  for (int r = 0; r < 4; ++r) bst.store(d9, 8, r, g == 0 ? (r == 0 ? dzs : dzc[r - 1]) : 0.0f);
  float bin[16][4];
  {
    const uint2 mk = *mask16_ptr(masks, blk, 8, half, lane);
    const float* w10 = tail + kBwdTailW10;
#pragma unroll
    for (int t = 0; t < 8; ++t) {
      const int fb = 16 * t + 4 * g;
      const f32x4 wa = *reinterpret_cast<const f32x4*>(w10 + fb);
      const f32x4 wb = *reinterpret_cast<const f32x4*>(w10 + 128 + fb);
      const f32x4 wc = *reinterpret_cast<const f32x4*>(w10 + 256 + fb);
      float v[4];
#pragma unroll
      for (int r = 0; r < 4; ++r)
        v[r] = mask16_apply(mk, t, r, __builtin_fmaf(wc[r], dzc[2], __builtin_fmaf(wb[r], dzc[1], wa[r] * dzc[0])));
      put_tile<P >= 2, true>(bin, t, v, bst, d9);
    }
  }
  if (tid < 64) reinterpret_cast<f32x4*>(w8_lds)[tid] = reinterpret_cast<const f32x4*>(tail + kBwdTailW8)[tid];
  __syncthreads();

  int cur = 0;
  const float* wsrc = a.wimg_b;
  f32x4 accA[16], accB[16];
  AE* delta_blk = reinterpret_cast<AE*>(a.delta) + (size_t)blk * kWidth * kBlk;
  BwdEpi16<true, ST, P >= 2> e7(accA, bin, bst, lane);
  e7.begin(mask16_ptr(masks, blk, 7, half, lane), delta_blk + 7 * layer_stride, w8_lds, dzs);
  layer16<P, 4, 0, 16>(bin, nullptr, accA, lds, cur, wsrc, false, tid, lane);
  e7.tile01();
  BwdEpi16<false, ST, P >= 2> ea(accA, bin, bst, lane), eb(accB, bin, bst, lane);
  eb.begin(mask16_ptr(masks, blk, 6, half, lane), delta_blk + 6 * layer_stride);
  layer16<P, 8, 0, 16>(bin, nullptr, accB, lds, cur, wsrc, false, tid, lane, e7);
  eb.tile01();
  static_assert(kDepth == 8, "bwd pairing assumes 8 trunk layers");
  for (int l = kDepth - 2; l >= 2; l -= 2) {
    ea.begin(mask16_ptr(masks, blk, l - 1, half, lane), delta_blk + (l - 1) * layer_stride);
    layer16<P, 8, 0, 16>(bin, nullptr, accA, lds, cur, wsrc, false, tid, lane, eb);
    ea.tile01();
    eb.begin(mask16_ptr(masks, blk, l - 2, half, lane), delta_blk + (l - 2) * layer_stride);
    layer16<P, 8, 0, 16>(bin, nullptr, accB, lds, cur, wsrc, l == 2, tid, lane, ea);
    eb.tile01();
  }
#pragma unroll
  for (int t = 2; t < 16; ++t) eb(t);
}

hipError_t launch_mlp_bwd16(const BwdArgs& a, hipStream_t st) {
  const int nblk = a.M / kBlk;
  if (a.split == 2) hipLaunchKernelGGL(k_mlp_bwd16<2>, dim3((nblk + 3) / 4), dim3(kMlp16Threads), 0, st, a);
  else if (a.split == 3) hipLaunchKernelGGL(k_mlp_bwd16<3>, dim3((nblk + 3) / 4), dim3(kMlp16Threads), 0, st, a);
  else hipLaunchKernelGGL(k_mlp_bwd16<0>, dim3((nblk + 3) / 4), dim3(kMlp16Threads), 0, st, a);
  return hipGetLastError();
}

NOF_CHECK_UNIT(check_unit_mlp_bwd16)

}
```

### nerf-or-nothing_amd/csrc/kernels/mlp_fwd16.hip

```cpp
#include "common.h"
#include "geometry.h"
#include "launch.h"
#include "mlp16.h"

namespace nof {


template <bool store, bool kDensity, int NT, class ST, bool kSplit = false>
struct FwdEpi16 {
  static constexpr int kVmPerPart = store ? 4 : 0;
  const f32x4 (&acc)[16];
  float (&bin)[16][4];
  const ST& bst;
  const int g;
  const float* w8;
  __amdgpu_buffer_rsrc_t act_blk;
  uint2* mask_dst;
  uint32_t mw[2];
  f32x4 wnext;
  float zs;

  __device__ __forceinline__ FwdEpi16(const f32x4 (&acc_)[16], float (&bin_)[16][4], const ST& bst_, int lane)
      : acc(acc_), bin(bin_), bst(bst_), g(lane >> 4) {}
  template <class E>
  __device__ __forceinline__ void begin(E* act_blk_, uint2* mask_dst_, const float* w8_ = nullptr) {
    act_blk = blk_rsrc_t(act_blk_);
    mask_dst = mask_dst_;
    mw[0] = mw[1] = 0u;
    if constexpr (kDensity) {
      w8 = w8_ + 4 * g;
      wnext = *reinterpret_cast<const f32x4*>(w8);
      zs = 0.0f;
    }
  }
  __device__ __forceinline__ void operator()(int t) {
    const bool more = t + 1 < NT;
    f32x4 w4;
    if constexpr (kDensity) {
      w4 = wnext;
      if (more) wnext = *reinterpret_cast<const f32x4*>(w8 + 16 * (t + 1));
    }
    float hv[4];
#pragma unroll
    for (int r = 0; r < 4; ++r) {
      hv[r] = relu_bit(acc[t][r], mw[t >> 3]);
      if constexpr (kDensity) zs = __builtin_fmaf(w4[r], hv[r], zs);
    }
    put_tile<kSplit, store>(bin, t, hv, bst, act_blk);
    if constexpr (store && kVmPerPart > 0)
      if (!more) *mask_dst = make_uint2(mw[0], mw[1]);
  }
  __device__ __forceinline__ void tile01() {
    (*this)(0);
    (*this)(1);
  }
};

template <int P, bool store>
__global__ __launch_bounds__(kMlp16Threads, 1) void k_mlp_fwd16(FwdArgs a) {
  typedef typename Store16<P, false>::T ST;
  typedef typename Store16<P, false>::E AE;
  constexpr int kRing = ring16_slots<P>() * kSliceFloats;
  constexpr bool kIpeReg = ring16_slots<P>() == 4;
  constexpr int kIpeLds = kIpeReg ? 0 : 8 * kIpe16Floats;
  constexpr int kBiasLds = 8 * 256 + 256;
  __shared__ __attribute__((aligned(16))) float lds[kRing + kIpeLds + 8 * 128 + kBiasLds];
  const int tid = threadIdx.x, lane = tid & 63, g = lane >> 4, j = lane & 15;
  const int wave = __builtin_amdgcn_readfirstlane(tid >> 6);
  const int half = wave & 1;
  const int nblk = a.M / kBlk;
  const int blk_raw = blockIdx.x * 4 + (wave >> 1);
  const int blk = blk_raw < nblk ? blk_raw : nblk - 1;
  const int m0 = blk * kBlk;
  const int ray = m0 / a.S;
  const int s0 = m0 - ray * a.S + 16 * half;
  const int m = m0 + 16 * half + j;
  const float* tail = a.wimg + (size_t)kFwdSlices * kSliceFloats;
  NOF_DCHECK(a.M % kBlk == 0 && a.S % kBlk == 0 && blk >= 0 && blk < nblk, kChkMlpBlock);

  ring16_prologue(a.wimg, lds, tid);

  float ipe[6][4];
  float d3[3];
  if (!a.encoded) {
    d3[0] = a.dirs[3 * ray]; d3[1] = a.dirs[3 * ray + 1]; d3[2] = a.dirs[3 * ray + 2];
    const float o3[3] = {a.origins[3 * ray], a.origins[3 * ray + 1], a.origins[3 * ray + 2]};
    const float* tr = a.t + (size_t)ray * (a.S + 1) + s0 + j;
    float mean[3], cov[3];
    frustum_gaussian(tr[0], tr[1], o3, d3, a.radii[ray], mean, cov, a.cylinder != 0);
#pragma unroll
    for (int t = 0; t < 6; ++t)
#pragma unroll
      for (int r = 0; r < 4; ++r)
        ipe[t][r] = ipe_feature(feat16(t, g, r), mean, cov);
  } else {
#pragma unroll
    for (int t = 0; t < 6; ++t)
#pragma unroll
      for (int r = 0; r < 4; ++r) ipe[t][r] = a.enc_pos[(size_t)m * kPosIn + feat16(t, g, r)];
  }
  const int kl = lane < kDirIn ? lane : 0;
  const float pe_l = a.encoded ? a.enc_dir[(size_t)ray * kDirIn + kl] : dir_feature(kl, d3);
  float pe[kDirIn];
#pragma unroll
  for (int k = 0; k < kDirIn; ++k) pe[k] = __int_as_float(__builtin_amdgcn_readlane(__float_as_int(pe_l), k));

  const ST bst(lane, half);
  if constexpr (store) {
    const __amdgpu_buffer_rsrc_t act_in_rs = blk_rsrc_t(reinterpret_cast<AE*>(a.act_in) + (size_t)blk * kInF * kBlk);
#pragma unroll
    for (int t = 0; t < 6; ++t)
#pragma unroll
      for (int r = 0; r < 4; ++r) bst.store(act_in_rs, t, r, ipe[t][r]);
#pragma unroll
    for (int t = 6; t < 8; ++t)
#pragma unroll
      for (int r = 0; r < 4; ++r) {
        const int k = feat16(t, g, r) - kPosIn;
        float v = 0.0f;
#pragma unroll
        for (int kk = 0; kk < kDirIn; ++kk) v = (kk == k) ? pe[kk] : v;
        bst.store(act_in_rs, t, r, v);
      }
  }
  const float* ipe_b = &ipe[0][0];
  if constexpr (!kIpeReg) {
    float* ipe_lds = lds + kRing + wave * kIpe16Floats;
#pragma unroll
    for (int t = 0; t < 6; ++t) {
      f32x4 v;
      v[0] = ipe[t][0]; v[1] = ipe[t][1]; v[2] = ipe[t][2]; v[3] = ipe[t][3];
      *reinterpret_cast<f32x4*>(ipe_lds + (t * 64 + lane) * 4) = v;
    }
    ipe_b = ipe_lds;
  }
  float* dirb = lds + kRing + kIpeLds + wave * 128;
  float* bias_lds = lds + kRing + kIpeLds + 8 * 128;
  for (int i = tid; i < kBiasLds / 4; i += kMlp16Threads) {
    const float* src = i < 512 ? tail + kFwdTailBias + 4 * i : tail + kFwdTailW8 + 4 * (i - 512);
    *reinterpret_cast<f32x4*>(bias_lds + 4 * i) = *reinterpret_cast<const f32x4*>(src);
  }
#pragma unroll
  for (int rep = 0; rep < 2; ++rep) {
    const int o = lane + 64 * rep;
    float s = tail[kFwdTailBias + 9 * 256 + o];
    const float* w9 = tail + kFwdTailW9d + o * 32;
#pragma unroll
    for (int k = 0; k < kDirIn; ++k) s = __builtin_fmaf(w9[k], pe[k], s);
    dirb[o] = s;
  }
  __syncthreads();

  int cur = 0;
  const float* wsrc = a.wimg;
  f32x4 accA[16], accB[16];
  float bin[16][4];
  const size_t layer_stride = (size_t)nblk * kWidth * kBlk;
  const float* biases = bias_lds;
  AE* act_h_blk = reinterpret_cast<AE*>(a.act_h) + (size_t)blk * kWidth * kBlk;

  constexpr bool kPre = P >= 2;
  FwdEpi16<store, false, 16, ST, kPre> ea(accA, bin, bst, lane), eb(accB, bin, bst, lane);
  const float* bias_g = biases + 4 * g;
  ea.begin(act_h_blk, mask16_ptr(a.masks, blk, 0, half, lane));
  layer16<P, 0, 3, 16>(bin, ipe_b, accA, lds, cur, wsrc, false, tid, lane, bias_g);
  ea.tile01();
  for (int l = 1; l < kDepth - 1; l += 2) {
    eb.begin(act_h_blk + l * layer_stride, mask16_ptr(a.masks, blk, l, half, lane));
    layer16<P, 8, 0, 16>(bin, ipe_b, accB, lds, cur, wsrc, false, tid, lane, ea, bias_g + l * 256);
    eb.tile01();
    ea.begin(act_h_blk + (l + 1) * layer_stride, mask16_ptr(a.masks, blk, l + 1, half, lane));
    if (l + 1 == kSkip)
      layer16<P, 8, 3, 16>(bin, ipe_b, accA, lds, cur, wsrc, false, tid, lane, eb, bias_g + (l + 1) * 256);
    else layer16<P, 8, 0, 16>(bin, ipe_b, accA, lds, cur, wsrc, false, tid, lane, eb, bias_g + (l + 1) * 256);
    ea.tile01();
  }
  static_assert(kDepth == 8 && kSkip % 2 == 0, "trunk pairing assumes 8 layers and an even skip layer");
  FwdEpi16<store, true, 16, ST, kPre> e7(accB, bin, bst, lane);
  e7.begin(act_h_blk + 7 * layer_stride, mask16_ptr(a.masks, blk, 7, half, lane), bias_lds + 8 * 256);
  layer16<P, 8, 0, 16>(bin, ipe_b, accB, lds, cur, wsrc, false, tid, lane, ea, bias_g + 7 * 256);
  e7.tile01();

  layer16<P, 8, 0, 8>(bin, ipe_b, accA, lds, cur, wsrc, true, tid, lane, e7, dirb + 4 * g);
  float zs = e7.zs;
  zs += __shfl_xor(zs, 16, 64);
  zs += __shfl_xor(zs, 32, 64);
  zs += tail[kFwdTailBias + 8 * 256];
  FwdEpi16<store, false, 8, ST> e9(accA, bin, bst, lane);
  e9.begin(reinterpret_cast<AE*>(a.act_h9) + (size_t)blk * kWidthCond * kBlk, mask16_ptr(a.masks, blk, 8, half, lane));
#pragma unroll
  for (int t = 0; t < 8; ++t) e9(t);

  float zc[3] = {0.0f, 0.0f, 0.0f};
#pragma unroll
  for (int c = 0; c < 3; ++c) {
#pragma unroll
    for (int t = 0; t < 8; ++t) {
      const f32x4 w4 = *reinterpret_cast<const f32x4*>(tail + kFwdTailW10 + c * 128 + 16 * t + 4 * g);
#pragma unroll
      for (int r = 0; r < 4; ++r) zc[c] = __builtin_fmaf(w4[r], bin[t][r], zc[c]);
    }
    zc[c] += __shfl_xor(zc[c], 16, 64);
    zc[c] += __shfl_xor(zc[c], 32, 64);
    zc[c] += tail[kFwdTailBias + 10 * 256 + c];
  }

  if (g == 0) {
    a.sigma[m] = softplus_f(zs + a.dbias);
#pragma unroll
    for (int c = 0; c < 3; ++c) a.rgb[(size_t)m * 3 + c] = sigmoid_f(zc[c]) * a.rgb_scale - a.rgb_pad;
    f32x4 zh;
    zh[0] = zs; zh[1] = zc[0]; zh[2] = zc[1]; zh[3] = zc[2];
    if constexpr (store) reinterpret_cast<f32x4*>(a.zhead)[m] = zh;
  }
}

hipError_t launch_mlp_fwd16(const FwdArgs& a, hipStream_t st) {
  const int nblk = a.M / kBlk;
  const dim3 grid((nblk + 3) / 4), block(kMlp16Threads);
  if (a.split == 2) {
    if (a.no_store) hipLaunchKernelGGL((k_mlp_fwd16<2, false>), grid, block, 0, st, a);
    else hipLaunchKernelGGL((k_mlp_fwd16<2, true>), grid, block, 0, st, a);
  } else if (a.split == 3) {
    if (a.no_store) hipLaunchKernelGGL((k_mlp_fwd16<2, false>), grid, block, 0, st, a);
    else hipLaunchKernelGGL((k_mlp_fwd16<3, true>), grid, block, 0, st, a);
  } else {
    if (a.no_store) hipLaunchKernelGGL((k_mlp_fwd16<0, false>), grid, block, 0, st, a);
    else hipLaunchKernelGGL((k_mlp_fwd16<0, true>), grid, block, 0, st, a);
  }
  return hipGetLastError();
}

NOF_CHECK_UNIT(check_unit_mlp_fwd16)

// ... 2 lines not shown
```

### nerf-or-nothing_amd/nof/__init__.py

```python
from ._lib import NofError, default_config, lib
from .api import (
    AcceleratedAdamOptimizer,
    AcceleratedGradientCalculator,
    AcceleratedMipNeRF,
    AcceleratedMLP,
    OutputRetriever,
    RayDataset,
    load_checkpoint,
    recenter_poses,
    save_checkpoint,
    device_checks,
    device_checks_selftest,
    device_count,
    device_tensor,
    gen_dispatch_h_names,
    gen_dispatch_names,
    generate_rays,
    grad_bucket_spans,
    image_metrics,
    kernel_gemm_h,
    kernel_interlevel,
    learning_rate_decay,
    multiscale_layout,
    to_numpy,
)
```

### nerf-or-nothing_amd/nof/_lib.py

```python
from __future__ import annotations

import ctypes as C
import os

_PKG = os.path.dirname(os.path.dirname(os.path.abspath(__file__)))
LIB_PATH = os.environ.get("NOF_LIB") or os.path.join(_PKG, "lib", "libnof.so")

NOF_MAX_LEVELS = 4
NOF_NUM_TIMERS = 8
TIMER_NAMES = ("pack", "sample", "mlp_fwd", "render_fwd", "render_bwd", "mlp_bwd", "wgrad", "wgrad_reduce")
STATUS = {0: "NOF_OK", 1: "NOF_ERR_INVALID_ARG", 2: "NOF_ERR_HIP", 3: "NOF_ERR_RCCL", 4: "NOF_ERR_OOM",
          5: "NOF_ERR_UNSUPPORTED"}


class NofError(RuntimeError):
    def __init__(self, status: int, where: str, msg: str):
        super().__init__(f"{where}: {STATUS.get(status, status)}: {msg}")
        self.status = status


NOF_PRECISION_F32, NOF_PRECISION_F32_SPLIT, NOF_PRECISION_F16X2, NOF_PRECISION_F32_F16SPLIT, NOF_PRECISION_F16 = 0, 1, 2, 3, 4
NOF_PRECISION_F16_PRODUCTS = 5
PRECISION_NAMES = {"f32": NOF_PRECISION_F32, "split": NOF_PRECISION_F32_SPLIT, "f16x2": NOF_PRECISION_F16X2,
                   "f16split": NOF_PRECISION_F32_F16SPLIT, "f16": NOF_PRECISION_F16,
# ... 44 lines not shown


class nof_gemm_src(C.Structure):
    _fields_ = [("p", C.c_void_p), ("si", C.c_int64), ("sk", C.c_int64), ("idiv", C.c_int32)]


class nof_gemm_args(C.Structure):
    _fields_ = [("M", C.c_int32), ("N", C.c_int32), ("K1", C.c_int32), ("K2", C.c_int32),
                ("A1", nof_gemm_src), ("A2", nof_gemm_src), ("B1", nof_gemm_src), ("B2", nof_gemm_src),
                ("bias", C.c_void_p), ("relu", C.c_int32), ("G", C.c_void_p), ("gi", C.c_int64), ("gj", C.c_int64),
                ("C", C.c_void_p), ("ci", C.c_int64), ("cj", C.c_int64), ("kchunk", C.c_int32),
                ("slab_stride", C.c_int64), ("rowsum", C.c_void_p), ("scale_amax", C.c_void_p),
                ("scale_src", C.c_int32), ("ksplit", C.c_int32)]


class nof_render_out(C.Structure):
    _fields_ = [("num_levels", C.c_int32), ("comp_rgb", C.c_void_p * NOF_MAX_LEVELS),
                ("distance", C.c_void_p * NOF_MAX_LEVELS), ("acc", C.c_void_p * NOF_MAX_LEVELS)]


class nof_batch(C.Structure):
    _fields_ = [("n", C.c_int32)] + [(k, C.c_void_p) for k in (
        "origins", "directions", "viewdirs", "radii", "nears", "fars", "loss_mults", "pixels", "record_index")]


class nof_step_stats(C.Structure):
    _fields_ = [(k, C.c_float) for k in ("weight_l2", "grad_norm", "grad_abs_max", "grad_norm_clipped",
                                         "clip_scale")] + [("iteration", C.c_int32)]


class nof_view_out(C.Structure):
    _fields_ = [("rgb", C.c_void_p * NOF_MAX_LEVELS), ("distance", C.c_void_p), ("acc", C.c_void_p)]


class nof_view_metrics(C.Structure):
    _fields_ = [("width", C.c_int32), ("height", C.c_int32), ("num_levels", C.c_int32),
                ("mse", C.c_double * NOF_MAX_LEVELS), ("psnr", C.c_float * NOF_MAX_LEVELS), ("ssim", C.c_float)]


NOF_VIEW_SSIM = 1

OUTPUT_GRAD_FN = C.CFUNCTYPE(C.c_uint64, C.c_void_p, C.c_uint64, C.c_int32, C.c_float, C.c_uint64)
GRAD_BUCKET_FN = C.CFUNCTYPE(None, C.c_void_p, C.c_int32, C.c_int32, C.POINTER(C.c_int64), C.POINTER(C.c_int64))
NOF_GRAD_ACCUMULATE, NOF_GRAD_PUBLISH, NOF_GRAD_BUCKETS = 1, 2, 2
NOF_NUMERIC_FORWARD, NOF_NUMERIC_DELTA = 1, 2

P = C.c_void_p
F = C.c_float
I32 = C.c_int32
U32 = C.c_uint32
U64 = C.c_uint64
PP = C.POINTER(C.POINTER(C.c_float))

SIGNATURES = {
    "nof_config_default": [C.POINTER(nof_config)],
    "nof_last_error": [],
    "nof_version": [],
    "nof_config_size": [],
    "nof_mipnerf_create": [C.POINTER(nof_config), C.POINTER(P)],
    "nof_mipnerf_create_ex": [C.POINTER(nof_config), C.POINTER(nof_model_ext), C.POINTER(P)],
    "nof_mipnerf_appearance": [P, C.POINTER(P), C.POINTER(P), C.POINTER(I32), C.POINTER(I32)],
    "nof_mipnerf_set_ray_views": [P, P],
    "nof_mipnerf_set_render_appearance": [P, I32],
    "nof_mipnerf_destroy": [P],
    "nof_mipnerf_get_gradient": [P, I32, P, P, P, P, P, P, OUTPUT_GRAD_FN, P, C.POINTER(PP)],
    "nof_mipnerf_get_gradient_device": [P, I32, P, P, P, P, P, P, P, F, C.POINTER(PP)],
    "nof_mipnerf_get_gradient_device_ex": [P, I32, P, P, P, P, P, P, P, F, U32, C.POINTER(PP)],
    "nof_mipnerf_set_grad_buckets": [P, GRAD_BUCKET_FN, P],
    "nof_grad_bucket_spans": [I32, C.POINTER(I32), I32, C.POINTER(C.c_int64), C.POINTER(C.c_int64),
                              C.POINTER(I32)],
    "nof_mipnerf_layer_sizes": [P, C.POINTER(I32), I32, C.POINTER(I32)],
    "nof_mipnerf_mlp": [P, C.POINTER(P)],
    "nof_mipnerf_set_rng": [P, U64, U32, U32],
    "nof_mipnerf_get_rng": [P, C.POINTER(U64), C.POINTER(U32), C.POINTER(U32)],
    "nof_mipnerf_level_view": [P, I32, C.POINTER(nof_level_view)],
    "nof_mipnerf_cross_view": [P, I32, C.POINTER(P), C.POINTER(P)],
    "nof_mipnerf_set_ray_grad": [P, I32],
    "nof_mipnerf_ray_grad": [P, C.POINTER(P), C.POINTER(P)],
    "nof_mipnerf_loss": [P, C.POINTER(F)],
    "nof_mipnerf_distortion_loss": [P, C.POINTER(F)],
    "nof_mipnerf_set_interlevel_loss": [P, F],
    "nof_mipnerf_set_contraction": [P, I32],
    "nof_mipnerf_get_contraction": [P, P],
    "nof_mipnerf_interlevel_loss": [P, C.POINTER(F)],
    "nof_mipnerf_numeric_status": [P, C.POINTER(U32), I32],
    "nof_device_checks": [C.POINTER(U32), I32],
    "nof_device_checks_selftest": [],
    "nof_mipnerf_render_device": [P, I32, P, P, P, P, P, I32, I32, C.POINTER(nof_render_out)],
    "nof_image_metrics": [P, P, I32, I32, F, C.POINTER(F), C.POINTER(F), P],
    "nof_dataset_open": [C.c_char_p, I32, C.POINTER(P)],
    "nof_dataset_open_streaming": [C.c_char_p, I32, C.c_int64, C.POINTER(P)],
    "nof_dataset_is_streaming": [P, C.POINTER(I32)],
    "nof_dataset_from_host": [P, C.c_int64, I32, C.POINTER(P)],
    "nof_dataset_count": [P, C.POINTER(C.c_int64)],
    "nof_dataset_next": [P, I32, U64, U32, U32, P, C.POINTER(nof_batch), C.POINTER(F)],
    "nof_dataset_destroy": [P],
    "nof_generate_rays": [P, I32, I32, I32, F, F, F, I32, P, P, P],
    "nof_dataset_generate": [P, I32, I32, I32, F, F, F, I32, P, I32, C.POINTER(P)],
    "nof_multiscale_layout": [I32, I32, F, I32, I32, I32, C.POINTER(I32), C.POINTER(I32), C.POINTER(F),
                              C.POINTER(F), C.POINTER(C.c_int64), C.POINTER(C.c_int64)],
    "nof_dataset_from_images": [P, I32, I32, I32, F, F, F, I32, P, I32, I32, I32, C.POINTER(P)],
    "nof_dataset_materialize": [P, P, P],
    "nof_dataset_scene_info": [P, C.POINTER(I32), C.POINTER(I32), C.POINTER(I32), C.POINTER(I32), C.POINTER(I32)],
    "nof_dataset_render_view": [P, P, I32, P, I32, U32, C.POINTER(nof_view_out), C.POINTER(nof_view_metrics)],
    "nof_dataset_pose_grad": [P, I32, P, P, P, I32, P],
    "nof_dataset_batch_views": [P, I32, P, P],
    "nof_dataset_get_poses": [P, P],
    "nof_dataset_set_poses": [P, P],
    "nof_recenter_poses": [P, I32],
    "nof_dp_unique_id": [P],
    "nof_dp_init_rank": [P, I32, I32, I32, C.POINTER(P)],
    "nof_dp_init_rank_timeout": [P, I32, I32, I32, I32, C.POINTER(P)],
    "nof_dp_attach": [P, P, P],
    "nof_dp_wait": [P, I32],
    "nof_dp_step_end": [P, I32],
    "nof_dp_abort": [P],
    "nof_dp_init_all": [I32, C.POINTER(I32), C.POINTER(P)],
    "nof_dp_allreduce": [P, P, C.c_int64, P],
    "nof_dp_allreduce_grads": [P, P, P],
    "nof_dp_allreduce_grads_all": [I32, C.POINTER(P), C.POINTER(P), C.POINTER(P)],
    "nof_dp_destroy": [P],
    "nof_dp_init_loopback": [I32, I32, C.POINTER(P)],
    "nof_dp_train_step": [I32, C.POINTER(P), C.POINTER(P), C.POINTER(P), C.POINTER(P), I32, I32, U64, I32, F,
                          C.POINTER(F)],
    "nof_checkpoint_save": [C.c_char_p, P, P],
    "nof_checkpoint_load": [C.c_char_p, P, P],
    "nof_mipnerf_enable_timing": [P, I32],
    "nof_mipnerf_enable_timing_mask": [P, C.c_uint32],
    "nof_mipnerf_read_timing": [P, C.POINTER(F), C.POINTER(I32), I32],
    "nof_mlp_get_output": [P, P, P, I32, I32, I32, C.POINTER(U64), C.POINTER(U64)],
    "nof_mlp_get_gradient": [P, P, P, I32, C.POINTER(PP)],
    "nof_mlp_get_gradient_ex": [P, P, P, I32, U32, C.POINTER(PP)],
    "nof_mlp_params": [P, C.POINTER(PP)],
    "nof_mlp_grads": [P, C.POINTER(PP)],
    "nof_mlp_flat_params": [P, C.POINTER(P), C.POINTER(C.c_int64)],
    "nof_mlp_flat_grads": [P, C.POINTER(P), C.POINTER(C.c_int64)],
    "nof_mlp_layer_sizes": [P, C.POINTER(I32), I32, C.POINTER(I32)],
    "nof_mlp_debug_view": [P, I32, C.POINTER(nof_mlp_debug)],
    "nof_mlp_gen_dispatch": [P, I32, C.POINTER(U32), I32, C.POINTER(I32)],
    "nof_gen_dispatch_name": [I32, C.POINTER(C.c_char_p)],
    "nof_mlp_gen_dispatch_h": [P, I32, C.POINTER(U32), I32, C.POINTER(I32)],
    "nof_gen_dispatch_h_name": [I32, C.POINTER(C.c_char_p)],
    "nof_adam_create": [C.POINTER(I32), I32, C.POINTER(nof_config), C.POINTER(P)],
    "nof_adam_step": [P, PP, PP, F],
    "nof_adam_iteration": [P, C.POINTER(I32)],
    "nof_adam_destroy": [P],
    "nof_adam_set_options": [P, F, F, F, I32],
    "nof_adam_get_options": [P, C.POINTER(F), C.POINTER(F), C.POINTER(F), C.POINTER(I32)],
    "nof_adam_stats": [P, C.POINTER(nof_step_stats)],
    "nof_adam_moments": [P, C.POINTER(P), C.POINTER(P), C.POINTER(C.c_int64)],
    "nof_gradcalc_create": [I32, C.POINTER(nof_config), C.POINTER(P)],
    "nof_gradcalc_output_gradient": [P, U64, P, I32, U64, F, I32, C.POINTER(U64)],
    "nof_gradcalc_destroy": [P],
    "nof_retrieve_output": [U64, I32, P],
    "nof_lr_decay": [I32, F, F, I32, I32, F],
    "nof_device_count": [C.POINTER(I32)],
    "nof_set_device": [I32],
    "nof_malloc": [C.POINTER(P), C.c_size_t],
    "nof_free": [P],
    "nof_memcpy_h2d": [P, P, C.c_size_t],
    "nof_memcpy_d2h": [P, P, C.c_size_t],
    "nof_memcpy_d2d": [P, P, C.c_size_t, P],
    "nof_memset": [P, C.c_int, C.c_size_t],
    "nof_stream_sync": [P],
    "nof_kernel_sample_stratified": [I32, I32, P, P, I32, U64, U32, U32, U32, P, P],
    "nof_kernel_sample_stratified_ex": [I32, I32, P, P, I32, U64, U32, U32, U32, P, P, I32],
# ... 79 lines not shown
```

### nerf-or-nothing_amd/nof/api.py

```python
from __future__ import annotations

import ctypes as C

import numpy as np

from . import _lib as L
from ._lib import call, lib


def _f32(a):
    return np.ascontiguousarray(a, dtype=np.float32)


def _ptr(x) -> int:
    if x is None:
        return 0
    if isinstance(x, int):
        return x
    return int(x.data_ptr())


def device_tensor(ptr: int, shape, dtype="float32", device=None):
    import torch

    typestr = {"float32": "<f4", "int32": "<i4"}[dtype]
    n = int(np.prod(shape))

    class _View:
        __cuda_array_interface__ = {"shape": (n,), "typestr": typestr, "data": (int(ptr), False), "version": 3}

    dev = device if device is not None else torch.device("cuda", torch.cuda.current_device())
    return torch.as_tensor(_View(), device=dev).view(*shape)


def to_numpy(ptr: int, shape, dtype=np.float32) -> np.ndarray:
    out = np.empty(shape, dtype)
    call("nof_memcpy_d2h", out.ctypes.data, C.c_void_p(ptr), out.nbytes)
    return out


def _ptr_list(pp, count) -> list[int]:
    return [C.cast(pp[i], C.c_void_p).value or 0 for i in range(count)]


def gen_dispatch_names() -> list[str]:
    out, name = [], C.c_char_p()
    while lib().nof_gen_dispatch_name(len(out), C.byref(name)) == 0:
        out.append(name.value.decode())
    return out


def gen_dispatch_h_names() -> list[str]:
    out, name = [], C.c_char_p()
    while lib().nof_gen_dispatch_h_name(len(out), C.byref(name)) == 0:
        out.append(name.value.decode())
    return out


def kernel_gemm_h(stream=None, **fields) -> None:
    a = L.nof_gemm_args()
    a.ksplit = 1
    for k, v in fields.items():
        if k in ("A1", "A2", "B1", "B2"):
            src = getattr(a, k)
            src.p, src.si, src.sk = _ptr(v[0]), int(v[1]), int(v[2])
            src.idiv = int(v[3]) if len(v) > 3 else 1
        elif k in ("bias", "G", "C", "rowsum", "scale_amax"):
            setattr(a, k, None if v is None else _ptr(v))
        else:
            setattr(a, k, int(v))
    call("nof_kernel_gemm_h", C.byref(a), stream)


def kernel_interlevel(n, samples_prop, t_prop, w_prop, samples_tgt, t_tgt, w_tgt, loss_mults, loss_mult_sum, mult,
                      w_grad, rays=None, accumulate=False, stream=None) -> None:
    call("nof_kernel_interlevel", int(n), int(samples_prop), _ptr(t_prop), _ptr(w_prop), int(samples_tgt),
         _ptr(t_tgt), _ptr(w_tgt), _ptr(loss_mults), float(loss_mult_sum), float(mult), int(bool(accumulate)),
         _ptr(w_grad), _ptr(rays) or None, stream)


class AcceleratedMLP:

    NUM_TENSORS = 22

    def __init__(self, handle, owner):
        self._h = handle
        self._owner = owner
        self.num_tensors = len(self.get_layer_sizes())

    def get_layer_sizes(self) -> list[int]:
# ... 178 lines not shown
            st = lib().nof_mipnerf_get_gradient_device_ex(*args, flags, C.byref(pp))
        if self._hook_errors:
            raise self._hook_errors[0]
        L.check(st, "nof_mipnerf_get_gradient_device")
        return _ptr_list(pp, self.mlp.num_tensors)

    def set_grad_buckets(self, fn):
        if fn is None:
            self._bucket_cb = None
            call("nof_mipnerf_set_grad_buckets", self._h, L.GRAD_BUCKET_FN(), None)
            return

        def tramp(user, bucket, nspans, offs, cnts):
            try:
                fn(int(bucket), [(int(offs[i]), int(cnts[i])) for i in range(nspans)])
            except Exception as e:
                self._hook_errors.append(e)

        self._bucket_cb = L.GRAD_BUCKET_FN(tramp)
        call("nof_mipnerf_set_grad_buckets", self._h, self._bucket_cb, None)

    def GetLayerSizes(self) -> list[int]:
        out = (C.c_int32 * 64)()
        cnt = C.c_int32()
        call("nof_mipnerf_layer_sizes", self._h, out, 64, C.byref(cnt))
        return list(out[: cnt.value])

    def set_rng(self, seed: int, step: int, ray_base: int = 0):
        call("nof_mipnerf_set_rng", self._h, seed, step, ray_base)

    def get_rng(self):
        s, st, rb = C.c_uint64(), C.c_uint32(), C.c_uint32()
        call("nof_mipnerf_get_rng", self._h, C.byref(s), C.byref(st), C.byref(rb))
        return s.value, st.value, rb.value

    def level_view(self, level: int) -> dict:
        v = L.nof_level_view()
        call("nof_mipnerf_level_view", self._h, level, C.byref(v))
        n, S = v.n, v.samples
        shapes = {"t": (n, S + 1), "weights": (n, S), "comp_rgb": (n, 3), "density": (n, S), "rgb": (n, S, 3),
                  "density_grad": (n, S), "rgb_grad": (n, S, 3)}
        return {k: (getattr(v, k), shp) for k, shp in shapes.items()}

    def level_numpy(self, level: int) -> dict:
        return {k: to_numpy(p, shp) for k, (p, shp) in self.level_view(level).items()}

    def cross_numpy(self, level: int) -> dict:
        v = L.nof_level_view()
        call("nof_mipnerf_level_view", self._h, level, C.byref(v))
        q, dt = C.c_void_p(), C.c_void_p()
        call("nof_mipnerf_cross_view", self._h, level, C.byref(q), C.byref(dt))
        return {"w_grad": to_numpy(q.value, (v.n, v.samples)) if q.value else None,
                "t_grad": to_numpy(dt.value, (v.n, v.samples + 1)) if dt.value else None}

    def set_ray_grad(self, on: bool = True) -> None:
        call("nof_mipnerf_set_ray_grad", self._h, int(bool(on)))

    def ray_grad(self):
        o, d = C.c_void_p(), C.c_void_p()
        call("nof_mipnerf_ray_grad", self._h, C.byref(o), C.byref(d))
        return o.value, d.value

    def loss(self) -> float:
        out = C.c_float()
        call("nof_mipnerf_loss", self._h, C.byref(out))
        return out.value

    def distortion_loss(self) -> float:
        out = C.c_float()
        call("nof_mipnerf_distortion_loss", self._h, C.byref(out))
        return out.value

    def set_interlevel_loss(self, mult: float) -> None:
        call("nof_mipnerf_set_interlevel_loss", self._h, float(mult))

    def interlevel_loss(self) -> float:
        out = C.c_float()
        call("nof_mipnerf_interlevel_loss", self._h, C.byref(out))
        return out.value

    def set_contraction(self, mode=1) -> None:
        call("nof_mipnerf_set_contraction", self._h, int(mode))

    def contraction(self) -> int:
        out = C.c_int32()
        call("nof_mipnerf_get_contraction", self._h, C.byref(out))
        return out.value

    def appearance(self):
        t, g, V, G = C.c_void_p(), C.c_void_p(), C.c_int32(), C.c_int32()
        call("nof_mipnerf_appearance", self._h, C.byref(t), C.byref(g), C.byref(V), C.byref(G))
        return t.value, g.value, V.value, G.value

    def set_ray_views(self, view_ids) -> None:
        call("nof_mipnerf_set_ray_views", self._h, _ptr(view_ids) or None)

    def set_render_appearance(self, view: int = -1) -> None:
        call("nof_mipnerf_set_render_appearance", self._h, int(view))

    def numeric_status(self, clear: bool = True) -> int:
        out = C.c_uint32()
        call("nof_mipnerf_numeric_status", self._h, C.byref(out), int(clear))
        return out.value

    def render_device(self, n, origins, directions, radii, nears, fars, randomized=False, white_bkgd=None):
        out = L.nof_render_out()
        white = self.config.white_bkgd if white_bkgd is None else int(white_bkgd)
        call("nof_mipnerf_render_device", self._h, n, _ptr(origins), _ptr(directions), _ptr(radii), _ptr(nears),
             _ptr(fars), int(randomized), white, C.byref(out))
        return [{"comp_rgb": (out.comp_rgb[l], (n, 3)), "distance": (out.distance[l], (n,)),
                 "acc": (out.acc[l], (n,))} for l in range(out.num_levels)]

    def render_rays(self, rays: dict, randomized=False, chunk=None, device=None) -> list[dict]:
        import torch

        dev = device or torch.device("cuda", self.config.device)
        N = rays["o"].shape[0]
        chunk = min(chunk or self.config.max_rays, self.config.max_rays)
        keys = ("o", "d", "radius", "near", "far")
        outs = None
        for b in range(0, N, chunk):
            e = min(N, b + chunk)
            t = {k: torch.from_numpy(np.ascontiguousarray(rays[k][b:e], dtype=np.float32)).to(dev) for k in keys}
            lv = self.render_device(e - b, t["o"], t["d"], t["radius"], t["near"], t["far"], randomized)
            torch.cuda.synchronize(dev)
            res = [{k: to_numpy(p, shp) for k, (p, shp) in L_.items()} for L_ in lv]
            if outs is None:
                outs = [{k: [] for k in r} for r in res]
            for o, r in zip(outs, res):
                for k, v in r.items():
                    o[k].append(v)
        return [{k: np.concatenate(v) for k, v in o.items()} for o in outs]

    def enable_timing(self, on: bool = True, timers=None):
        if timers is None:
            call("nof_mipnerf_enable_timing", self._h, int(on))
        else:
            mask = sum(1 << L.TIMER_NAMES.index(t) for t in timers) if on else 0
            call("nof_mipnerf_enable_timing_mask", self._h, C.c_uint32(mask))

    def read_timing(self) -> dict:
        ms = (C.c_float * L.NOF_NUM_TIMERS)()
        cnt = (C.c_int32 * L.NOF_NUM_TIMERS)()
        call("nof_mipnerf_read_timing", self._h, ms, cnt, L.NOF_NUM_TIMERS)
        return {name: (ms[i], cnt[i]) for i, name in enumerate(L.TIMER_NAMES)}


class AcceleratedAdamOptimizer:

    def __init__(self, layer_sizes, config: L.nof_config | None = None, grad_max_norm: float = 0.0,
                 grad_max_val: float = 0.0, weight_decay_mult: float = 0.0, stats: bool = False):
        self.config = config if config is not None else L.default_config()
        arr = (C.c_int32 * len(layer_sizes))(*layer_sizes)
        self.n = len(layer_sizes)
        h = C.c_void_p()
        call("nof_adam_create", arr, len(layer_sizes), C.byref(self.config), C.byref(h))
        self._h = h
        if grad_max_norm or grad_max_val or weight_decay_mult or stats:
            self.set_options(grad_max_norm, grad_max_val, weight_decay_mult, stats)

    def set_options(self, grad_max_norm: float = 0.0, grad_max_val: float = 0.0, weight_decay_mult: float = 0.0,
                    stats: bool = False):
        call("nof_adam_set_options", self._h, float(grad_max_norm), float(grad_max_val), float(weight_decay_mult),
             int(bool(stats)))

    def get_options(self) -> dict:
# ... 300 lines not shown
```

Baseline: 164,000 rays/s.

## Precompute per-ray view tables in pack kernel and pair backward levels in f32

The weight-pack kernel gains extra blocks that compute each ray's direction encoding and its layer-9 directional bias once, and the forward kernel reads these tables instead of recomputing them per sample block. The f32/split precision paths now run two levels in a single backward launch, and the backward and forward prologues hoist their global loads ahead of the weight-ring prologue, replacing __syncthreads with explicit waitcnt barriers. The aim is fewer launches, less redundant per-block work, and better latency hiding. It costs extra buffers and hand-coded wait counts that could break if the store counts change.

```diff
diff --git a/include/nof.h b/include/nof.h
--- a/include/nof.h
+++ b/include/nof.h
@@ -118,6 +118,8 @@
 enum { NOF_CONTRACT_NONE = 0, NOF_CONTRACT_SPHERE = 1 };
 nof_status nof_mipnerf_set_contraction(nof_mipnerf* h, int32_t mode);
 nof_status nof_mipnerf_get_contraction(nof_mipnerf* h, int32_t* mode);
+enum { NOF_STEP_FUSION_BWD_PAIR = 1, NOF_STEP_FUSION_VIEW_TABLES = 2, NOF_STEP_FUSION_ALL = 3 };
+nof_status nof_mipnerf_set_step_fusion(nof_mipnerf* h, uint32_t flags);
 typedef struct nof_model_ext {
   uint32_t size;
   int32_t appearance_views, appearance_dim;
diff --git a/nerf-or-nothing_amd/csrc/capi.cpp b/nerf-or-nothing_amd/csrc/capi.cpp
--- a/nerf-or-nothing_amd/csrc/capi.cpp
+++ b/nerf-or-nothing_amd/csrc/capi.cpp
@@ -293,6 +293,12 @@
     h->impl->set_contraction(mode);
   });
 }
+nof_status nof_mipnerf_set_step_fusion(nof_mipnerf* h, uint32_t flags) {
+  return guard([&] {
+    ARG(h && (flags & ~(uint32_t)NOF_STEP_FUSION_ALL) == 0);
+    h->impl->mlp->set_step_fusion(flags);
+  });
+}
 nof_status nof_mipnerf_get_contraction(nof_mipnerf* h, int32_t* mode) {
   return guard([&] { ARG(h && mode); *mode = h->impl->contraction(); });
 }
diff --git a/nerf-or-nothing_amd/csrc/host/accelerated.cpp b/nerf-or-nothing_amd/csrc/host/accelerated.cpp
--- a/nerf-or-nothing_amd/csrc/host/accelerated.cpp
+++ b/nerf-or-nothing_amd/csrc/host/accelerated.cpp
@@ -225,6 +225,8 @@
     NOF_HIP(hipMemset(L.delta9x.p, 0, L.delta9x.n * sizeof(float)));
     max_M_ = std::max(max_M_, L.cap);
   }
+  view_pe_.alloc((size_t)cfg.max_rays * 32);
+  view_bias_.alloc((size_t)cfg.max_rays * 128);
   slab_cap_ = (size_t)(num_cu_ + 64) * 65536;
   slabs_.alloc(slab_cap_);
   bias_slabs_.alloc((size_t)(num_cu_ + 64) * 256);
@@ -237,7 +239,9 @@
   return s;
 }
 
-bool AcceleratedMLP::pack_weights(const nof::StratArgs* strat) {
+bool AcceleratedMLP::pack_weights(const nof::StratArgs* strat, const float* view_dirs, int view_n) {
+  view_dirs_ = nullptr;
+  view_n_ = 0;
   if (generic_) {
     if (f16_products()) {
       NOF_HIP(hipMemsetAsync(amax_.p, 0, lv_.size() * sizeof(uint32_t), st_));
@@ -254,6 +258,13 @@
     pa.nzero = (int)lv_.size();
     amax_cleared_ = (1u << lv_.size()) - 1u;
     amax_given_ = 0u;
+  }
+  const bool fwd16 = precision_ == NOF_PRECISION_F32 || precision_ == NOF_PRECISION_F16X2 ||
+                     precision_ == NOF_PRECISION_F32_F16SPLIT;
+  if (view_dirs && view_n > 0 && view_n <= cfg_.max_rays && fwd16 && (step_fusion_ & NOF_STEP_FUSION_VIEW_TABLES)) {
+    pa.view.n = view_n; pa.view.dirs = view_dirs; pa.view.pe = view_pe_.p; pa.view.bias = view_bias_.p;
+    view_dirs_ = view_dirs;
+    view_n_ = view_n;
   }
   tb(kTPack);
   if (precision_ == NOF_PRECISION_F16)
@@ -318,6 +329,10 @@
   a.no_store = inference ? 1 : 0;
   a.cylinder = cfg_.ray_shape == NOF_RAY_CYLINDRICAL ? 1 : 0;
   a.t = t; a.origins = origins; a.dirs = dirs; a.radii = radii;
+  if (view_dirs_ && view_dirs_ == dirs && n <= view_n_) {
+    a.view_pe = view_pe_.p;
+    a.view_bias = view_bias_.p;
+  }
   run_forward(level, a);
 }
 
@@ -751,7 +766,10 @@
   else
     for (int b = 0; b < kBuckets; ++b) (void)schedule(0, nl, b);
   int l = 0;
-  if (precision_ == NOF_PRECISION_F16)
+  const bool pair16 = (step_fusion_ & NOF_STEP_FUSION_BWD_PAIR) &&
+                      (precision_ == NOF_PRECISION_F32 || precision_ == NOF_PRECISION_F16X2 ||
+                       precision_ == NOF_PRECISION_F32_F16SPLIT);
+  if (precision_ == NOF_PRECISION_F16 || pair16)
     for (; l + 1 < nl; l += 2) run_backward2(l, color_grads + l, density_grads + l);
   for (; l < nl; ++l) run_backward(l, color_grads[l], density_grads[l]);
   return wgrad_levels(0, nl, (flags & NOF_GRAD_ACCUMULATE) ? 1 : 0, buckets);
@@ -1294,7 +1312,7 @@
   nof::StratArgs sa;
   sa.n = n; sa.S = cfg_.num_samples[0]; sa.nears = nears; sa.fars = fars; sa.randomized = cfg_.randomized;
   sa.lindisp = cfg_.lindisp; sa.seed = seed_; sa.step = step_; sa.ray_base = ray_base_; sa.t = t_[0].p;
-  const bool sampled = mlp->pack_weights(&sa);
+  const bool sampled = mlp->pack_weights(&sa, d, n);
   for (int lv = 0; lv < L; ++lv) {
     TraceRange lr(kFwd[lv & 3]);
     const int S = cfg_.num_samples[lv];
diff --git a/nerf-or-nothing_amd/csrc/host/accelerated.h b/nerf-or-nothing_amd/csrc/host/accelerated.h
--- a/nerf-or-nothing_amd/csrc/host/accelerated.h
+++ b/nerf-or-nothing_amd/csrc/host/accelerated.h
@@ -117,7 +117,7 @@
 
   void forward_fused(int level, int n, int samples, const float* t, const float* origins, const float* dirs,
                      const float* radii, bool inference = false);
-  bool pack_weights(const nof::StratArgs* strat = nullptr);
+  bool pack_weights(const nof::StratArgs* strat = nullptr, const float* view_dirs = nullptr, int view_n = 0);
   const float* density(int level) const { return lv_[level].sigma.p; }
   const float* rgb(int level) const { return lv_[level].rgb.p; }
   KernelTimer* timer = nullptr;
@@ -158,6 +158,8 @@
   void set_appearance_job(const int32_t* ids, int accumulate, int levels) {
     app_job_ = AppJob{ids, accumulate, levels, true};
   }
+  void set_step_fusion(uint32_t flags) { step_fusion_ = flags; }
+  uint32_t step_fusion() const { return step_fusion_; }
 
  private:
   struct AppJob {
@@ -199,6 +201,10 @@
   hipStream_t st_;
   int num_cu_ = 256;
   int precision_ = 0;
+#ifndef NOF_STEP_FUSION_DEFAULT
+#define NOF_STEP_FUSION_DEFAULT NOF_STEP_FUSION_ALL
+#endif
+  uint32_t step_fusion_ = NOF_STEP_FUSION_DEFAULT;
   bool f16_pieces() const {
     return precision_ == NOF_PRECISION_F16X2 || precision_ == NOF_PRECISION_F32_F16SPLIT || precision_ == NOF_PRECISION_F16;
   }
@@ -253,6 +259,9 @@
   static void gen_split(int nout, int ncols, int M, int* ksplit, int* kchunk);
   float* const* gen_publish(bool buckets);
   DevBuf<float> params_, grads_, wimg_f_, wimg_b_;
+  DevBuf<float> view_pe_, view_bias_;
+  const float* view_dirs_ = nullptr;
+  int view_n_ = 0;
   std::vector<float*> param_views_, grad_views_;
   std::vector<Level> lv_;
   int max_M_ = 0;
diff --git a/nerf-or-nothing_amd/csrc/kernels/adam.hip b/nerf-or-nothing_amd/csrc/kernels/adam.hip
--- a/nerf-or-nothing_amd/csrc/kernels/adam.hip
+++ b/nerf-or-nothing_amd/csrc/kernels/adam.hip
@@ -1,4 +1,5 @@
 #include "common.h"
+#include "geometry.h"
 #include "launch.h"
 #include "resample.h"
 #include "mlp_common.h"
@@ -9,6 +10,7 @@
 namespace nof {
 
 static int strat_blocks(const StratArgs& z) { return z.n > 0 ? (z.n * (z.S + 1) + 255) / 256 : 0; }
+static int view_blocks(const ViewTabArgs& v) { return v.n > 0 ? (v.n + 1) / 2 : 0; }
 
 __global__ void k_adam(int64_t n, float* __restrict__ p, const float* __restrict__ g, float* __restrict__ m,
                        float* __restrict__ v, float lr, float inv1, float inv2) {
@@ -191,14 +193,40 @@
   else { l = 7 - (s - 4) / 8; o = 32 * ((s - 4) % 8); }
 }
 
+__device__ inline bool pack_extra_block(const float* __restrict__ P, const PackArgs& pa) {
+  const int xb = (int)blockIdx.x - pa.pack_blocks;
+  if (xb < 0) return false;
+  if (xb < pa.strat_blocks) {
+    const StratArgs& z = pa.strat;
+    stratified_t(xb * (int)blockDim.x + (int)threadIdx.x, z.n, z.S, z.nears, z.fars, z.randomized, z.lindisp, z.seed,
+                 z.step, 0, z.ray_base, z.t);
+    return true;
+  }
+  __shared__ float pe_s[2][32];
+  const ViewTabArgs& v = pa.view;
+  const int sub = (int)threadIdx.x >> 7, o = (int)threadIdx.x & 127;
+  const int ray = 2 * (xb - pa.strat_blocks) + sub;
+  const bool live = ray < v.n;
+  if (live && o < 32) {
+    const float d3[3] = {v.dirs[3 * ray], v.dirs[3 * ray + 1], v.dirs[3 * ray + 2]};
+    const float f = o < kDirIn ? dir_feature(o, d3) : 0.0f;
+    pe_s[sub][o] = f;
+    v.pe[(size_t)ray * 32 + o] = f;
+  }
+  __syncthreads();
+  if (live) {
+    float s = P[pa.boff[9] + o];
+    const float* w9 = P + pa.woff[9] + (int64_t)o * 283 + 256;
+#pragma unroll
+    for (int k = 0; k < kDirIn; ++k) s = __builtin_fmaf(w9[k], pe_s[sub][k], s);
+    v.bias[(size_t)ray * 128 + o] = s;
+  }
+  return true;
+}
+
 __global__ void k_pack_weights(const float* __restrict__ P, PackArgs pa, float* __restrict__ wf,
                                float* __restrict__ wb) {
-  if ((int)blockIdx.x >= pa.pack_blocks) {
-    const StratArgs& z = pa.strat;
-    stratified_t(((int)blockIdx.x - pa.pack_blocks) * (int)blockDim.x + (int)threadIdx.x, z.n, z.S, z.nears, z.fars,
-                 z.randomized, z.lindisp, z.seed, z.step, 0, z.ray_base, z.t);
-    return;
-  }
+  if (pack_extra_block(P, pa)) return;
   const int64_t gid = (int64_t)blockIdx.x * blockDim.x + threadIdx.x;
   const int64_t nf = (int64_t)kFwdImageFloats, nb = (int64_t)kBwdImageFloats;
   if (gid < nf) {
@@ -274,12 +302,7 @@
 template <int P>
 __global__ void k_pack_weights_x3(const float* __restrict__ P_, PackArgs pa, float* __restrict__ wf,
                                   float* __restrict__ wb) {
-  if ((int)blockIdx.x >= pa.pack_blocks) {
-    const StratArgs& z = pa.strat;
-    stratified_t(((int)blockIdx.x - pa.pack_blocks) * (int)blockDim.x + (int)threadIdx.x, z.n, z.S, z.nears, z.fars,
-                 z.randomized, z.lindisp, z.seed, z.step, 0, z.ray_base, z.t);
-    return;
-  }
+  if (pack_extra_block(P_, pa)) return;
   constexpr int NP = SplitMode<P>::NP;
   constexpr int kChunks = split_slice_floats<P>() / 4;
   const float* __restrict__ Pp = P_;
@@ -322,7 +345,8 @@
   const int64_t total = (int64_t)(kFwdSlices + kBwdSlices) * chunks + kFwdTail + kBwdTail;
   PackArgs a = pa;
   a.pack_blocks = (int)((total + 255) / 256);
-  const dim3 grid((unsigned)(a.pack_blocks + strat_blocks(pa.strat)));
+  a.strat_blocks = strat_blocks(pa.strat);
+  const dim3 grid((unsigned)(a.pack_blocks + a.strat_blocks + view_blocks(pa.view)));
   if (precision == 2) hipLaunchKernelGGL(k_pack_weights_x3<2>, grid, dim3(256), 0, st, params, a, wimg_f, wimg_b);
   else hipLaunchKernelGGL(k_pack_weights_x3<1>, grid, dim3(256), 0, st, params, a, wimg_f, wimg_b);
   return hipGetLastError();
@@ -392,9 +416,10 @@
   const int64_t total = (int64_t)kFwdImageFloats + (int64_t)kBwdImageFloats;
   PackArgs a = pa;
   a.pack_blocks = (int)((total + 255) / 256);
-  hipLaunchKernelGGL(k_pack_weights, dim3((unsigned)(a.pack_blocks + strat_blocks(pa.strat))), dim3(256), 0, st,
-                     params, a, wimg_f, wimg_b);
-  return hipGetLastError();
-}
-
-}
+  a.strat_blocks = strat_blocks(pa.strat);
+  hipLaunchKernelGGL(k_pack_weights, dim3((unsigned)(a.pack_blocks + a.strat_blocks + view_blocks(pa.view))),
+                     dim3(256), 0, st, params, a, wimg_f, wimg_b);
+  return hipGetLastError();
+}
+
+}
diff --git a/nerf-or-nothing_amd/csrc/kernels/launch.h b/nerf-or-nothing_amd/csrc/kernels/launch.h
--- a/nerf-or-nothing_amd/csrc/kernels/launch.h
+++ b/nerf-or-nothing_amd/csrc/kernels/launch.h
@@ -133,6 +133,7 @@
   float dbias = -1.0f, rgb_scale = 1.002f, rgb_pad = 0.001f;
   const float *t, *origins, *dirs, *radii;
   const float *enc_pos, *enc_dir;
+  const float *view_pe, *view_bias;
   const float* wimg;
   float* act_in;
   float* act_h;
@@ -370,11 +371,17 @@
   uint32_t step = 0, ray_base = 0;
   float* t = nullptr;
 };
+struct ViewTabArgs {
+  int n = 0;
+  const float* dirs = nullptr;
+  float *pe = nullptr, *bias = nullptr;
+};
 struct PackArgs {
   int woff[11]; int boff[11];
   uint32_t* zero = nullptr; int nzero = 0;
   StratArgs strat;
-  int pack_blocks = 0;
+  ViewTabArgs view;
+  int pack_blocks = 0, strat_blocks = 0;
 };
 hipError_t launch_pack_weights(const float* params, const PackArgs& pa, float* wimg_f, float* wimg_b, hipStream_t st);
 hipError_t launch_pack_weights_h32(const float* params, const PackArgs& pa, float* wimg_f, float* wimg_b,
diff --git a/nerf-or-nothing_amd/csrc/kernels/mlp_bwd16.hip b/nerf-or-nothing_amd/csrc/kernels/mlp_bwd16.hip
--- a/nerf-or-nothing_amd/csrc/kernels/mlp_bwd16.hip
+++ b/nerf-or-nothing_amd/csrc/kernels/mlp_bwd16.hip
@@ -52,7 +52,7 @@
 };
 
 template <int P>
-__global__ __launch_bounds__(kMlp16Threads, 1) void k_mlp_bwd16(BwdArgs a) {
+__global__ __launch_bounds__(kMlp16Threads, 1) void k_mlp_bwd16(BwdArgs a0) {
   typedef typename Store16<P, true>::T ST;
   typedef typename Store16<P, true>::E AE;
   __shared__ __attribute__((aligned(16))) float lds[ring16_floats<P>() + 256];
@@ -61,8 +61,28 @@
   const int wave = __builtin_amdgcn_readfirstlane(tid >> 6);
   const int half = wave & 1;
   const ST bst(lane, half);
+  const int wg0 = (a0.M / kBlk + 3) / 4;
+  const bool second = a0.M1 > 0 && (int)blockIdx.x >= wg0;
+  struct {
+    int M;
+    const float *dsigma, *drgb, *zhead;
+    const uint32_t *amax, *masks;
+    const float* wimg_b;
+    float dbias, rgb_scale;
+    float *delta, *delta9x;
+  } a;
+  a.M = second ? a0.M1 : a0.M;
+  a.dsigma = second ? a0.dsigma1 : a0.dsigma;
+  a.drgb = second ? a0.drgb1 : a0.drgb;
+  a.zhead = second ? a0.zhead1 : a0.zhead;
+  a.amax = second ? a0.amax1 : a0.amax;
+  a.masks = second ? a0.masks1 : a0.masks;
+  a.delta = second ? a0.delta1 : a0.delta;
+  a.delta9x = second ? a0.delta9x1 : a0.delta9x;
+  a.wimg_b = a0.wimg_b; a.dbias = a0.dbias; a.rgb_scale = a0.rgb_scale;
+  const int wg = second ? (int)blockIdx.x - wg0 : (int)blockIdx.x;
   const int nblk = a.M / kBlk;
-  const int blk_raw = blockIdx.x * 4 + (wave >> 1);
+  const int blk_raw = wg * 4 + (wave >> 1);
   const int blk = blk_raw < nblk ? blk_raw : nblk - 1;
   const int m = blk * kBlk + 16 * half + j;
   NOF_DCHECK(a.M % kBlk == 0 && blk >= 0 && blk < nblk, kChkMlpBlock);
@@ -70,44 +90,53 @@
   const size_t layer_stride = (size_t)nblk * kWidth * kBlk;
   uint32_t* masks = const_cast<uint32_t*>(a.masks);
 
+  const f32x4 zh = reinterpret_cast<const f32x4*>(a.zhead)[m];
+  const float dsig = a.dsigma[m];
+  const float drgb3[3] = {a.drgb[(size_t)m * 3], a.drgb[(size_t)m * 3 + 1], a.drgb[(size_t)m * 3 + 2]};
+  float sc = 1.0f;
+  if constexpr (P >= 2) sc = delta_scale(a.amax, false);
+  const uint2 mk9 = *mask16_ptr(masks, blk, 8, half, lane);
+  f32x4 w10r[8][3];
+#pragma unroll
+  for (int t = 0; t < 8; ++t)
+#pragma unroll
+    for (int c = 0; c < 3; ++c)
+      w10r[t][c] = *reinterpret_cast<const f32x4*>(tail + kBwdTailW10 + 128 * c + 16 * t + 4 * g);
+  const f32x4 w8r = reinterpret_cast<const f32x4*>(tail + kBwdTailW8)[lane];
+  __builtin_amdgcn_sched_barrier(0);
   ring16_prologue(a.wimg_b, lds, tid);
+  __builtin_amdgcn_sched_barrier(0);
 
-  const f32x4 zh = reinterpret_cast<const f32x4*>(a.zhead)[m];
-  float dzs = a.dsigma[m] * sigmoid_f(zh[0] + a.dbias);
+  float dzs = dsig * sigmoid_f(zh[0] + a.dbias);
   float dzc[3];
 #pragma unroll
   for (int c = 0; c < 3; ++c) {
     const float s = sigmoid_f(zh[1 + c]);
-    dzc[c] = a.drgb[(size_t)m * 3 + c] * (s * (1.0f - s)) * a.rgb_scale;
+    dzc[c] = drgb3[c] * (s * (1.0f - s)) * a.rgb_scale;
   }
   if constexpr (P >= 2) {
-    const float sc = delta_scale(a.amax, false);
     dzs *= sc;
 #pragma unroll
     for (int c = 0; c < 3; ++c) dzc[c] *= sc;
   }
+  if (wave == 0) reinterpret_cast<f32x4*>(w8_lds)[lane] = w8r;
   const __amdgpu_buffer_rsrc_t d9 = blk_rsrc_t(reinterpret_cast<AE*>(a.delta9x) + (size_t)blk * kD9F * kBlk);
 #pragma unroll
   for (int r = 0; r < 4; ++r) bst.store(d9, 8, r, g == 0 ? (r == 0 ? dzs : dzc[r - 1]) : 0.0f);
   float bin[16][4];
-  {
-    const uint2 mk = *mask16_ptr(masks, blk, 8, half, lane);
-    const float* w10 = tail + kBwdTailW10;
 #pragma unroll
-    for (int t = 0; t < 8; ++t) {
-      const int fb = 16 * t + 4 * g;
-      const f32x4 wa = *reinterpret_cast<const f32x4*>(w10 + fb);
-      const f32x4 wb = *reinterpret_cast<const f32x4*>(w10 + 128 + fb);
-      const f32x4 wc = *reinterpret_cast<const f32x4*>(w10 + 256 + fb);
-      float v[4];
+  for (int t = 0; t < 8; ++t) {
+    float v[4];
 #pragma unroll
-      for (int r = 0; r < 4; ++r)
-        v[r] = mask16_apply(mk, t, r, __builtin_fmaf(wc[r], dzc[2], __builtin_fmaf(wb[r], dzc[1], wa[r] * dzc[0])));
-      put_tile<P >= 2, true>(bin, t, v, bst, d9);
-    }
+    for (int r = 0; r < 4; ++r)
+      v[r] = mask16_apply(mk9, t, r, __builtin_fmaf(w10r[t][2][r], dzc[2],
+                                                   __builtin_fmaf(w10r[t][1][r], dzc[1], w10r[t][0][r] * dzc[0])));
+    put_tile<P >= 2, true>(bin, t, v, bst, d9);
   }
-  if (tid < 64) reinterpret_cast<f32x4*>(w8_lds)[tid] = reinterpret_cast<const f32x4*>(tail + kBwdTailW8)[tid];
-  __syncthreads();
+  constexpr int kD9Stores = 4 + 8 * (P == 2 ? 2 : 4);
+  static_assert(kD9Stores == (P == 2 ? 20 : 36), "the literals in the waits below");
+  if constexpr (P == 2) asm volatile("s_waitcnt vmcnt(20)\n\ts_waitcnt lgkmcnt(0)\n\ts_barrier" ::: "memory");
+  else asm volatile("s_waitcnt vmcnt(36)\n\ts_waitcnt lgkmcnt(0)\n\ts_barrier" ::: "memory");
 
   int cur = 0;
   const float* wsrc = a.wimg_b;
@@ -135,10 +164,10 @@
 }
 
 hipError_t launch_mlp_bwd16(const BwdArgs& a, hipStream_t st) {
-  const int nblk = a.M / kBlk;
-  if (a.split == 2) hipLaunchKernelGGL(k_mlp_bwd16<2>, dim3((nblk + 3) / 4), dim3(kMlp16Threads), 0, st, a);
-  else if (a.split == 3) hipLaunchKernelGGL(k_mlp_bwd16<3>, dim3((nblk + 3) / 4), dim3(kMlp16Threads), 0, st, a);
-  else hipLaunchKernelGGL(k_mlp_bwd16<0>, dim3((nblk + 3) / 4), dim3(kMlp16Threads), 0, st, a);
+  const dim3 grid((a.M / kBlk + 3) / 4 + (a.M1 > 0 ? (a.M1 / kBlk + 3) / 4 : 0));
+  if (a.split == 2) hipLaunchKernelGGL(k_mlp_bwd16<2>, grid, dim3(kMlp16Threads), 0, st, a);
+  else if (a.split == 3) hipLaunchKernelGGL(k_mlp_bwd16<3>, grid, dim3(kMlp16Threads), 0, st, a);
+  else hipLaunchKernelGGL(k_mlp_bwd16<0>, grid, dim3(kMlp16Threads), 0, st, a);
   return hipGetLastError();
 }
 
diff --git a/nerf-or-nothing_amd/csrc/kernels/mlp_fwd16.hip b/nerf-or-nothing_amd/csrc/kernels/mlp_fwd16.hip
--- a/nerf-or-nothing_amd/csrc/kernels/mlp_fwd16.hip
+++ b/nerf-or-nothing_amd/csrc/kernels/mlp_fwd16.hip
@@ -78,16 +78,37 @@
   const float* tail = a.wimg + (size_t)kFwdSlices * kSliceFloats;
   NOF_DCHECK(a.M % kBlk == 0 && a.S % kBlk == 0 && blk >= 0 && blk < nblk, kChkMlpBlock);
 
+  const bool vtab = a.view_pe != nullptr;
+  float t01[2] = {0.0f, 0.0f};
+  float d3[3] = {0.0f, 0.0f, 0.0f}, o3[3] = {0.0f, 0.0f, 0.0f}, radius = 0.0f;
+  if (!a.encoded) {
+    const float* tr = a.t + (size_t)ray * (a.S + 1) + s0 + j;
+    t01[0] = tr[0]; t01[1] = tr[1];
+    d3[0] = a.dirs[3 * ray]; d3[1] = a.dirs[3 * ray + 1]; d3[2] = a.dirs[3 * ray + 2];
+    o3[0] = a.origins[3 * ray]; o3[1] = a.origins[3 * ray + 1]; o3[2] = a.origins[3 * ray + 2];
+    radius = a.radii[ray];
+  }
+  f32x4 vpe[2] = {};
+  float vb[2] = {0.0f, 0.0f};
+  if (vtab) {
+#pragma unroll
+    for (int u = 0; u < 2; ++u)
+      vpe[u] = *reinterpret_cast<const f32x4*>(a.view_pe + (size_t)ray * 32 + (feat16(6 + u, g, 0) - kPosIn));
+#pragma unroll
+    for (int rep = 0; rep < 2; ++rep) vb[rep] = a.view_bias[(size_t)ray * 128 + lane + 64 * rep];
+  }
+  static_assert(kBiasLds / 4 > kMlp16Threads && kBiasLds / 4 <= kMlp16Threads + 64, "bias table: wave 0 takes the rest");
+  const f32x4 tab0 = *reinterpret_cast<const f32x4*>(tail + kFwdTailBias + 4 * tid);
+  f32x4 tab1 = {};
+  if (wave == 0) tab1 = *reinterpret_cast<const f32x4*>(tail + kFwdTailW8 + 4 * tid);
+  __builtin_amdgcn_sched_barrier(0);
   ring16_prologue(a.wimg, lds, tid);
+  __builtin_amdgcn_sched_barrier(0);
 
   float ipe[6][4];
-  float d3[3];
   if (!a.encoded) {
-    d3[0] = a.dirs[3 * ray]; d3[1] = a.dirs[3 * ray + 1]; d3[2] = a.dirs[3 * ray + 2];
-    const float o3[3] = {a.origins[3 * ray], a.origins[3 * ray + 1], a.origins[3 * ray + 2]};
-    const float* tr = a.t + (size_t)ray * (a.S + 1) + s0 + j;
     float mean[3], cov[3];
-    frustum_gaussian(tr[0], tr[1], o3, d3, a.radii[ray], mean, cov, a.cylinder != 0);
+    frustum_gaussian(t01[0], t01[1], o3, d3, radius, mean, cov, a.cylinder != 0);
 #pragma unroll
     for (int t = 0; t < 6; ++t)
 #pragma unroll
@@ -98,30 +119,17 @@
     for (int t = 0; t < 6; ++t)
 #pragma unroll
       for (int r = 0; r < 4; ++r) ipe[t][r] = a.enc_pos[(size_t)m * kPosIn + feat16(t, g, r)];
-  }
-  const int kl = lane < kDirIn ? lane : 0;
-  const float pe_l = a.encoded ? a.enc_dir[(size_t)ray * kDirIn + kl] : dir_feature(kl, d3);
+#pragma unroll
+    for (int t = 0; t < 6; ++t)
+#pragma unroll
+      for (int r = 0; r < 4; ++r) asm volatile("" : "+v"(ipe[t][r]));
+  }
   float pe[kDirIn];
-#pragma unroll
-  for (int k = 0; k < kDirIn; ++k) pe[k] = __int_as_float(__builtin_amdgcn_readlane(__float_as_int(pe_l), k));
-
-  const ST bst(lane, half);
-  if constexpr (store) {
-    const __amdgpu_buffer_rsrc_t act_in_rs = blk_rsrc_t(reinterpret_cast<AE*>(a.act_in) + (size_t)blk * kInF * kBlk);
-#pragma unroll
-    for (int t = 0; t < 6; ++t)
-#pragma unroll
-      for (int r = 0; r < 4; ++r) bst.store(act_in_rs, t, r, ipe[t][r]);
-#pragma unroll
-    for (int t = 6; t < 8; ++t)
-#pragma unroll
-      for (int r = 0; r < 4; ++r) {
-        const int k = feat16(t, g, r) - kPosIn;
-        float v = 0.0f;
-#pragma unroll
-        for (int kk = 0; kk < kDirIn; ++kk) v = (kk == k) ? pe[kk] : v;
-        bst.store(act_in_rs, t, r, v);
-      }
+  if (!vtab) {
+    const int kl = lane < kDirIn ? lane : 0;
+    const float pe_l = a.encoded ? a.enc_dir[(size_t)ray * kDirIn + kl] : dir_feature(kl, d3);
+#pragma unroll
+    for (int k = 0; k < kDirIn; ++k) pe[k] = __int_as_float(__builtin_amdgcn_readlane(__float_as_int(pe_l), k));
   }
   const float* ipe_b = &ipe[0][0];
   if constexpr (!kIpeReg) {
@@ -136,20 +144,59 @@
   }
   float* dirb = lds + kRing + kIpeLds + wave * 128;
   float* bias_lds = lds + kRing + kIpeLds + 8 * 128;
-  for (int i = tid; i < kBiasLds / 4; i += kMlp16Threads) {
-    const float* src = i < 512 ? tail + kFwdTailBias + 4 * i : tail + kFwdTailW8 + 4 * (i - 512);
-    *reinterpret_cast<f32x4*>(bias_lds + 4 * i) = *reinterpret_cast<const f32x4*>(src);
-  }
-#pragma unroll
-  for (int rep = 0; rep < 2; ++rep) {
-    const int o = lane + 64 * rep;
-    float s = tail[kFwdTailBias + 9 * 256 + o];
-    const float* w9 = tail + kFwdTailW9d + o * 32;
-#pragma unroll
-    for (int k = 0; k < kDirIn; ++k) s = __builtin_fmaf(w9[k], pe[k], s);
-    dirb[o] = s;
-  }
-  __syncthreads();
+  *reinterpret_cast<f32x4*>(bias_lds + 4 * tid) = tab0;
+  if (wave == 0) *reinterpret_cast<f32x4*>(bias_lds + 4 * (kMlp16Threads + tid)) = tab1;
+  if (vtab) {
+#pragma unroll
+    for (int rep = 0; rep < 2; ++rep) dirb[lane + 64 * rep] = vb[rep];
+  } else {
+#pragma unroll
+    for (int rep = 0; rep < 2; ++rep) {
+      const int o = lane + 64 * rep;
+      float s = tail[kFwdTailBias + 9 * 256 + o];
+      const float* w9 = tail + kFwdTailW9d + o * 32;
+#pragma unroll
+      for (int k = 0; k < kDirIn; ++k) s = __builtin_fmaf(w9[k], pe[k], s);
+      dirb[o] = s;
+    }
+  }
+
+  const ST bst(lane, half);
+  if constexpr (store) {
+    float vrow[2][4];
+    if (vtab) {
+#pragma unroll
+      for (int u = 0; u < 2; ++u)
+#pragma unroll
+        for (int r = 0; r < 4; ++r) vrow[u][r] = vpe[u][r];
+    } else {
+#pragma unroll
+      for (int u = 0; u < 2; ++u)
+#pragma unroll
+        for (int r = 0; r < 4; ++r) {
+          const int k = feat16(6 + u, g, r) - kPosIn;
+          float v = 0.0f;
+#pragma unroll
+          for (int kk = 0; kk < kDirIn; ++kk) v = (kk == k) ? pe[kk] : v;
+          vrow[u][r] = v;
+        }
+    }
+    __builtin_amdgcn_sched_barrier(0);
+    const __amdgpu_buffer_rsrc_t act_in_rs = blk_rsrc_t(reinterpret_cast<AE*>(a.act_in) + (size_t)blk * kInF * kBlk);
+#pragma unroll
+    for (int t = 0; t < 6; ++t)
+#pragma unroll
+      for (int r = 0; r < 4; ++r) bst.store(act_in_rs, t, r, ipe[t][r]);
+#pragma unroll
+    for (int u = 0; u < 2; ++u)
+#pragma unroll
+      for (int r = 0; r < 4; ++r) bst.store(act_in_rs, 6 + u, r, vrow[u][r]);
+    constexpr int kActInStores = 8 * 4;
+    static_assert(kActInStores == 32 && kActInStores < 64, "the literal in the wait below");
+    asm volatile("s_waitcnt vmcnt(32)\n\ts_waitcnt lgkmcnt(0)\n\ts_barrier" ::: "memory");
+  } else {
+    __syncthreads();
+  }
 
   int cur = 0;
   const float* wsrc = a.wimg;
diff --git a/nerf-or-nothing_amd/nof/__init__.py b/nerf-or-nothing_amd/nof/__init__.py
--- a/nerf-or-nothing_amd/nof/__init__.py
+++ b/nerf-or-nothing_amd/nof/__init__.py
@@ -1,5 +1,8 @@
 from ._lib import NofError, default_config, lib
 from .api import (
+    STEP_FUSION_ALL,
+    STEP_FUSION_BWD_PAIR,
+    STEP_FUSION_VIEW_TABLES,
     AcceleratedAdamOptimizer,
     AcceleratedGradientCalculator,
     AcceleratedMipNeRF,
diff --git a/nerf-or-nothing_amd/nof/_lib.py b/nerf-or-nothing_amd/nof/_lib.py
--- a/nerf-or-nothing_amd/nof/_lib.py
+++ b/nerf-or-nothing_amd/nof/_lib.py
@@ -150,6 +150,7 @@
     "nof_mipnerf_set_interlevel_loss": [P, F],
     "nof_mipnerf_set_contraction": [P, I32],
     "nof_mipnerf_get_contraction": [P, P],
+    "nof_mipnerf_set_step_fusion": [P, U32],
     "nof_mipnerf_interlevel_loss": [P, C.POINTER(F)],
     "nof_mipnerf_numeric_status": [P, C.POINTER(U32), I32],
     "nof_device_checks": [C.POINTER(U32), I32],
diff --git a/nerf-or-nothing_amd/nof/api.py b/nerf-or-nothing_amd/nof/api.py
--- a/nerf-or-nothing_amd/nof/api.py
+++ b/nerf-or-nothing_amd/nof/api.py
@@ -6,6 +6,10 @@
 
 from . import _lib as L
 from ._lib import call, lib
+
+STEP_FUSION_BWD_PAIR = 1
+STEP_FUSION_VIEW_TABLES = 2
+STEP_FUSION_ALL = 3
 
 
 def _f32(a):
@@ -350,6 +354,9 @@
     def set_contraction(self, mode=1) -> None:
         call("nof_mipnerf_set_contraction", self._h, int(mode))
 
+    def set_step_fusion(self, flags: int = STEP_FUSION_ALL) -> None:
+        call("nof_mipnerf_set_step_fusion", self._h, int(flags))
+
     def contraction(self) -> int:
         out = C.c_int32()
         call("nof_mipnerf_get_contraction", self._h, C.byref(out))
```

Measured after the change: 166,200 rays/s, median of 6. 1.3% higher.
